# comprna/radian

Measured on AMD Instinct MI355X. Metric: signal samples/s basecalled (chunk=1024, beam=10), higher is better.
Workload: dtype f32

## Files before the change

include/radian_hip.h:

```cpp
#ifndef RADIAN_HIP_H
#define RADIAN_HIP_H

#include <stddef.h>
#include <stdint.h>

#ifdef __cplusplus
extern "C" {
#endif

#define RD_OK 0
#define RD_ERR_ARG (-1)
#define RD_ERR_HIP (-2)
#define RD_ERR_STATE (-3)
#define RD_ERR_NOMEM (-4)
#define RD_ERR_RCCL (-5)
#define RD_ERR_FORMAT (-6)
#define RD_ERR_IO (-7)
#define RD_LEN_MISSING_CONTEXT (-1)

typedef struct rd_ctx rd_ctx;

const char* rd_last_error(void);
int rd_version(void);
int rd_device_count(int* n);
int rd_decode_max_width(void);
int rd_decode_lane_width(void);

int rd_create(int device_id, rd_ctx** out);
int rd_destroy(rd_ctx* ctx);
int rd_sync(rd_ctx* ctx);
int rd_set_precision(rd_ctx* ctx, int mode);

typedef struct rd_weights_header {
    uint32_t magic;
    uint32_t version;
    uint32_t nb_filters;
    uint32_t kernel_size;
    uint32_t relu_units;
    uint32_t n_classes;
    uint32_t n_blocks;
    uint32_t dilations[16];
    uint32_t n_floats;
} rd_weights_header;
int rd_load_weights(rd_ctx* ctx, const void* blob, size_t nbytes);

int rd_load_lm(rd_ctx* ctx, const double* table, int k);
int rd_load_lm_absent(rd_ctx* ctx, int k);
int rd_load_lm_hashed(rd_ctx* ctx, const double* table, int table_order, int context_len);
int rd_set_logits(rd_ctx* ctx, int mode);
int rd_set_decode_partition(rd_ctx* ctx, int cus_per_xcd);
int rd_set_decode_math(rd_ctx* ctx, int mode);
int rd_set_head_pack(rd_ctx* ctx, int on);
int rd_head_pack_active(rd_ctx* ctx);
int64_t rd_head_pack_tiles(rd_ctx* ctx);

int rd_forward(rd_ctx* ctx, const float* windows, int n_windows, int chunk_len, float* probs);

int rd_assemble(rd_ctx* ctx, const float* probs, int n_windows, int chunk_len, int pad, int step, double* out,
                int64_t out_cap, int64_t* n_rows, int* is_f64);

int rd_decode_batch(rd_ctx* ctx, const void* probs, int prob_is_f64, const int64_t* seq_off, const int32_t* seq_len,
                    int n_seq, int beam_width, int use_lm, double s_thr, double r_thr, uint8_t* labels_out,
                    const int64_t* label_off, int32_t* label_len, double* best_score);

int rd_basecall_chunk(rd_ctx* ctx, const float* windows, int n_windows, int chunk_len, const int32_t* valid_len,
                      int beam_width, uint8_t* labels_out, int32_t* label_len);

int rd_basecall_global(rd_ctx* ctx, const float* windows, int chunk_len, int step, const int32_t* read_win_off,
                       const int32_t* pad, int n_reads, int beam_width, int use_lm, double s_thr, double r_thr,
                       uint8_t* labels_out, const int64_t* label_off, int32_t* label_len);

int rd_count_windows(int64_t n_samples, int chunk_len, int step);
int rd_basecall_reads_chunk(rd_ctx* ctx, const float* signal, const int64_t* read_off, int n_reads, int chunk_len,
                            int step, int beam_width, uint8_t* labels_out, int32_t* label_len);
int rd_basecall_reads_global(rd_ctx* ctx, const float* signal, const int64_t* read_off, int n_reads, int chunk_len,
                             int step, int beam_width, int use_lm, double s_thr, double r_thr, uint8_t* labels_out,
                             const int64_t* label_off, int32_t* label_len);

int rd_normalise_reads(rd_ctx* ctx, const int16_t* raw, const int64_t* read_off, int n_reads, int outlier_clip,
                       float* norm_out , int32_t* status);
int rd_basecall_raw_chunk(rd_ctx* ctx, const int16_t* raw, const int64_t* read_off, int n_reads, int outlier_clip,
                          int chunk_len, int step, int beam_width, uint8_t* labels_out, int32_t* label_len, int32_t* status);
int rd_basecall_raw_global(rd_ctx* ctx, const int16_t* raw, const int64_t* read_off, int n_reads, int outlier_clip,
                           int chunk_len, int step, int beam_width, int use_lm, double s_thr, double r_thr,
                           uint8_t* labels_out, const int64_t* label_off, int32_t* label_len, int32_t* status);

int rd_dev_alloc(rd_ctx* ctx, size_t bytes, void** d_ptr);
int rd_dev_free(rd_ctx* ctx, void* d_ptr);
int rd_mem_info(rd_ctx* ctx, size_t* free_bytes, size_t* total_bytes);
int rd_memcpy_h2d(rd_ctx* ctx, void* d_dst, const void* src, size_t bytes);
int rd_memcpy_d2h(rd_ctx* ctx, void* dst, const void* d_src, size_t bytes);
int rd_forward_resident(rd_ctx* ctx, const float* d_windows, int n_windows, int chunk_len, float* d_probs);
int rd_forward_reads_resident(rd_ctx* ctx, const float* d_signal, const int64_t* read_off, int n_reads, int chunk_len,
                              int step, int decode_type, int lane, int64_t* total_rows);
int rd_forward_reads(rd_ctx* ctx, const float* signal, const int64_t* read_off, int n_reads, int chunk_len, int step,
                     float* probs_out, int64_t windows_cap, int64_t* n_windows);
int rd_basecall_chunk_resident(rd_ctx* ctx, const float* d_windows, int n_windows, int chunk_len,
                               const int32_t* valid_len, int beam_width, uint8_t* labels_out, int32_t* label_len);
int rd_decode_resident(rd_ctx* ctx, const float* d_probs, int n_windows, int chunk_len, const int32_t* valid_len,
                       int beam_width, uint8_t* labels_out, int32_t* label_len);

int rd_basecall_reads_chunk_resident(rd_ctx* ctx, const float* d_signal, const int64_t* read_off, int n_reads,
                                     int chunk_len, int step, int beam_width, uint8_t* labels_out, int32_t* label_len);
int rd_basecall_reads_global_resident(rd_ctx* ctx, const float* d_signal, const int64_t* read_off, int n_reads,
                                      int chunk_len, int step, int beam_width, int use_lm, double s_thr, double r_thr,
                                      uint8_t* labels_out, const int64_t* label_off, int32_t* label_len);

int rd_pipe_config(rd_ctx* ctx, int group_batches);
int rd_pipe_set_lanes(rd_ctx* ctx, int lanes);
int rd_pipe_submit(rd_ctx* ctx, const float* d_windows, int n_windows, int chunk_len, const int32_t* valid_len,
                   int beam_width, uint8_t* labels_out, int32_t* label_len);
int rd_pipe_submit_reads(rd_ctx* ctx, const float* d_signal, const int64_t* read_off, int n_reads, int chunk_len,
                         int step, int beam_width, uint8_t* labels_out, int32_t* label_len);
int rd_pipe_submit_reads_global(rd_ctx* ctx, const float* d_signal, const int64_t* read_off, int n_reads, int chunk_len,
                                int step, int beam_width, int use_lm, double s_thr, double r_thr, uint8_t* labels_out,
                                const int64_t* label_off, int32_t* label_len);
int rd_pipe_submit_raw_global(rd_ctx* ctx, const int16_t* raw, const int64_t* read_off, int n_reads, int outlier_clip,
                              int chunk_len, int step, int beam_width, int use_lm, double s_thr, double r_thr,
                              uint8_t* labels_out, const int64_t* label_off, int32_t* label_len, int32_t* status);
int rd_pipe_submit_raw_chunk(rd_ctx* ctx, const int16_t* raw, const int64_t* read_off, int n_reads, int outlier_clip,
                             int chunk_len, int step, int beam_width, uint8_t* labels_out, int32_t* label_len, int32_t* status);
int rd_pipe_progress(rd_ctx* ctx, int64_t wait_for, int64_t* delivered);
int rd_pipe_flush(rd_ctx* ctx);
int rd_pipe_submitted(rd_ctx* ctx, int64_t* submitted);

int rd_lm_json_probe(const char* buf, size_t n, int* k_out);
int rd_lm_json_fill(const char* buf, size_t n, int k, double* table, int64_t* n_entries, int64_t* n_contexts);
int rd_lm_json_write(const char* path, const double* table, int k, int64_t* n_rows, int64_t* n_bytes);

int rd_fasta_scan(const char* buf, size_t n, int field, const char* value, uint8_t* codes, int64_t* offsets, int64_t* counts);
int rd_lm_build(rd_ctx* ctx, const uint8_t* codes, const int64_t* offsets, int64_t n_records, int k, int as_written, int unseen, double alpha,
                double r_thr, int64_t cut, double* table_out, uint32_t* counts_out, int64_t* stats);
int rd_lm_score(rd_ctx* ctx, const uint8_t* codes, const int64_t* offsets, int64_t n_records, int as_written, double r_thr, int64_t cut,
                int64_t* stats, double* nll_sum);

typedef struct rd_fast5 rd_fast5;
int rd_fast5_open(const char* path, rd_fast5** out);
int rd_fast5_open_mem(const void* buf, size_t n, rd_fast5** out);
void rd_fast5_close(rd_fast5* f);
int rd_fast5_count(const rd_fast5* f, int64_t* n_reads);
int rd_fast5_lengths(rd_fast5* f, int64_t lo, int64_t hi, int64_t* n_samples);
int rd_fast5_read_batch(rd_fast5* f, int64_t lo, int64_t hi, int16_t* samples, int64_t cap, int64_t* offsets, char* ids, int id_stride);

int rd_stitch_chunk(const uint8_t* labels, const int32_t* label_len, int chunk_len, const int32_t* read_win_off, int n_reads,
                    uint8_t* seq_out, const int64_t* seq_off, int32_t* seq_len, int n_threads);

#define RD_ALIGN_OK 0
#define RD_ALIGN_CLIP_INDEX_ERROR 1
#define RD_ALIGN_EMPTY_AFTER_CLIP 2
#define RD_ALIGN_TOO_LARGE 3
int rd_align_batch(rd_ctx* ctx, const uint8_t* refs, const int64_t* ref_off, const uint8_t* reads, const int64_t* read_off, int n_pairs,
                   int match, int mismatch, int gap_open, int gap_extend, int64_t budget_bytes, int32_t* score, int32_t* counts,
                   int32_t* status, uint8_t* ops_out, const int64_t* ops_off, int32_t* ops_len);
int64_t rd_align_workspace_bytes(int64_t n, int64_t m);
int rd_align_clip_count(const uint8_t* ops, int64_t n_ops, const uint8_t* ref, const uint8_t* read, int32_t* counts, int32_t* status);

#define RD_CTCALIGN_OK 0
#define RD_CTCALIGN_NO_PATH 1
#define RD_CTCALIGN_TOO_LARGE 2
int rd_ctc_align_batch(rd_ctx* ctx, const void* probs, int prob_is_f64, const int64_t* seq_off, const int32_t* seq_len, int n_seq,
                       const uint8_t* labels, const int64_t* label_off, const int32_t* label_len, int64_t budget_bytes,
                       int32_t* first_step, int32_t* last_step, uint8_t* qual, double* score, int32_t* status);
int64_t rd_ctc_align_workspace_bytes(int64_t n_rows, int64_t n_labels);
int rd_basecall_raw_global_q(rd_ctx* ctx, const int16_t* raw, const int64_t* read_off, int n_reads, int outlier_clip, int chunk_len,
                             int step, int beam_width, int use_lm, double s_thr, double r_thr, uint8_t* labels_out,
                             const int64_t* label_off, int32_t* label_len, int32_t* status, int64_t budget_bytes, uint8_t* qual_out,
                             int32_t* first_step_out, int32_t* last_step_out, double* score_out, int32_t* align_status);

int rd_event_stats(rd_ctx* ctx, const int16_t* raw, const int64_t* read_off, int n_reads, const int32_t* first_step,
                   const int32_t* last_step, const int64_t* label_off, const int32_t* label_len, const int32_t* align_status,
                   int32_t* ev_start, int32_t* ev_end, int64_t* ev_sum, int64_t* ev_sumsq, int16_t* ev_min, int16_t* ev_max);
int rd_event_stats_host(const int16_t* raw, const int64_t* read_off, int n_reads, const int32_t* first_step, const int32_t* last_step,
                        const int64_t* label_off, const int32_t* label_len, const int32_t* align_status, int32_t* ev_start,
                        int32_t* ev_end, int64_t* ev_sum, int64_t* ev_sumsq, int16_t* ev_min, int16_t* ev_max);
int rd_resquiggle_raw(rd_ctx* ctx, const int16_t* raw, const int64_t* read_off, int n_reads, int outlier_clip, int chunk_len, int step,
                      const uint8_t* ref_labels, const int64_t* ref_off, const int32_t* ref_len, int64_t budget_bytes,
                      int32_t* first_step, int32_t* last_step, uint8_t* qual, double* score, int32_t* align_status, int32_t* read_status,
                      int32_t* ev_start, int32_t* ev_end, int64_t* ev_sum, int64_t* ev_sumsq, int16_t* ev_min, int16_t* ev_max);

#define RD_POLYA_OK 0
#define RD_POLYA_NONE 1
#define RD_POLYA_MAD_ZERO 2
#define RD_POLYA_SHORT 3
#define RD_POLYA_EMPTY 4
#define RD_POLYA_TOO_LARGE 5
int rd_polya_segment(rd_ctx* ctx, const int16_t* raw, const int64_t* read_off, int n_reads, int win, int flat_q, int use_level, int lo_q,
                     int hi_q, int max_gap, int64_t min_samples, int64_t search_limit, int64_t budget_bytes, int32_t* status,
                     int64_t* tail_start, int64_t* tail_end, int32_t* n_flat, int64_t* sum, int64_t* sumsq, int32_t* m2, int32_t* d4,
                     int32_t* n_candidates);
int rd_polya_segment_host(const int16_t* raw, const int64_t* read_off, int n_reads, int win, int flat_q, int use_level, int lo_q, int hi_q,
                          int max_gap, int64_t min_samples, int64_t search_limit, int32_t* status, int64_t* tail_start, int64_t* tail_end,
                          int32_t* n_flat, int64_t* sum, int64_t* sumsq, int32_t* m2, int32_t* d4, int32_t* n_candidates);
int64_t rd_polya_workspace_bytes(int64_t n_samples, int win);
int rd_polya_diag_windows(rd_ctx* ctx, const int16_t* raw, const int64_t* read_off, int n_reads, int win, int flat_q, int use_level, int lo_q,
                          int hi_q, int32_t* m2, int32_t* d4, uint64_t* thr, int32_t* win_sum, int64_t* win_sumsq, uint8_t* win_flat);

#define RD_SITE_OK 0
#define RD_SITE_ONE_SIDED 1
#define RD_SITE_DEEP 2
#define RD_SITE_TOO_LARGE 3
int rd_site_compare(rd_ctx* ctx, const uint32_t* site, const uint8_t* cond, const int16_t* value, int64_t n_events, uint32_t n_sites,
                    int64_t budget_bytes, int64_t capacity, uint32_t* out_site, int32_t* status, int64_t* n, int64_t* sum, int64_t* sumsq,
                    int32_t* vmin, int32_t* vmax, int32_t* med2, int64_t* u2, int64_t* ks_num, int32_t* ks_x, int64_t* tie, int64_t* n_out);
int rd_site_compare_host(const uint32_t* site, const uint8_t* cond, const int16_t* value, int64_t n_events, uint32_t n_sites, int64_t capacity,
                         uint32_t* out_site, int32_t* status, int64_t* n, int64_t* sum, int64_t* sumsq, int32_t* vmin, int32_t* vmax,
                         int32_t* med2, int64_t* u2, int64_t* ks_num, int32_t* ks_x, int64_t* tie, int64_t* n_out);
int64_t rd_site_workspace_bytes(int64_t n_events);
// ... 172 lines not shown
```

radian_amd/_lib.py:

```python
import ctypes
import os

HERE = os.path.dirname(os.path.abspath(__file__))
LIB_PATH = os.environ.get("RADIAN_HIP_LIB") or os.path.join(HERE, "libradian_hip.so")

c_i = ctypes.c_int
c_i32p = ctypes.POINTER(ctypes.c_int32)
c_i64 = ctypes.c_int64
c_i64p = ctypes.POINTER(ctypes.c_int64)
c_d = ctypes.c_double
c_dp = ctypes.POINTER(ctypes.c_double)
c_fp = ctypes.POINTER(ctypes.c_float)
c_u8p = ctypes.POINTER(ctypes.c_uint8)
c_u32 = ctypes.c_uint32
c_u64 = ctypes.c_uint64
c_vp = ctypes.c_void_p
c_sz = ctypes.c_size_t

SIGNATURES = {
    "rd_last_error": (ctypes.c_char_p, []),
    "rd_version": (c_i, []),
    "rd_device_count": (c_i, [ctypes.POINTER(c_i)]),
    "rd_decode_max_width": (c_i, []),
    "rd_decode_lane_width": (c_i, []),
    "rd_create": (c_i, [c_i, ctypes.POINTER(c_vp)]),
    "rd_destroy": (c_i, [c_vp]),
    "rd_sync": (c_i, [c_vp]),
    "rd_set_precision": (c_i, [c_vp, c_i]),
    "rd_load_weights": (c_i, [c_vp, c_vp, c_sz]),
    "rd_load_lm": (c_i, [c_vp, c_vp, c_i]),
    "rd_load_lm_absent": (c_i, [c_vp, c_i]),
    "rd_load_lm_hashed": (c_i, [c_vp, c_vp, c_i, c_i]),
    "rd_set_logits": (c_i, [c_vp, c_i]),
    "rd_set_decode_math": (c_i, [c_vp, c_i]),
    "rd_set_head_pack": (c_i, [c_vp, c_i]),
    "rd_head_pack_active": (c_i, [c_vp]),
    "rd_head_pack_tiles": (c_i64, [c_vp]),
    "rd_set_decode_partition": (c_i, [c_vp, c_i]),
    "rd_forward": (c_i, [c_vp, c_vp, c_i, c_i, c_vp]),
    "rd_assemble": (c_i, [c_vp, c_vp, c_i, c_i, c_i, c_i, c_vp, c_i64, c_i64p, ctypes.POINTER(c_i)]),
    "rd_decode_batch": (c_i, [c_vp, c_vp, c_i, c_vp, c_vp, c_i, c_i, c_i, c_d, c_d, c_vp, c_vp, c_vp, c_vp]),
    "rd_basecall_chunk": (c_i, [c_vp, c_vp, c_i, c_i, c_vp, c_i, c_vp, c_vp]),
    "rd_basecall_global": (c_i, [c_vp, c_vp, c_i, c_i, c_vp, c_vp, c_i, c_i, c_i, c_d, c_d, c_vp, c_vp, c_vp]),
    "rd_count_windows": (c_i, [c_i64, c_i, c_i]),
    "rd_basecall_reads_chunk": (c_i, [c_vp, c_vp, c_vp, c_i, c_i, c_i, c_i, c_vp, c_vp]),
    "rd_basecall_reads_global": (c_i, [c_vp, c_vp, c_vp, c_i, c_i, c_i, c_i, c_i, c_d, c_d, c_vp, c_vp, c_vp]),
    "rd_basecall_reads_chunk_resident": (c_i, [c_vp, c_vp, c_vp, c_i, c_i, c_i, c_i, c_vp, c_vp]),
    "rd_basecall_reads_global_resident": (c_i, [c_vp, c_vp, c_vp, c_i, c_i, c_i, c_i, c_i, c_d, c_d, c_vp, c_vp, c_vp]),
    "rd_pipe_submit_reads": (c_i, [c_vp, c_vp, c_vp, c_i, c_i, c_i, c_i, c_vp, c_vp]),
    "rd_pipe_submit_reads_global": (c_i, [c_vp, c_vp, c_vp, c_i, c_i, c_i, c_i, c_i, c_d, c_d, c_vp, c_vp, c_vp]),
    "rd_pipe_submit_raw_global": (c_i, [c_vp, c_vp, c_vp, c_i, c_i, c_i, c_i, c_i, c_i, c_d, c_d, c_vp, c_vp, c_vp, c_vp]),
    "rd_pipe_submit_raw_chunk": (c_i, [c_vp, c_vp, c_vp, c_i, c_i, c_i, c_i, c_i, c_vp, c_vp, c_vp]),
    "rd_pipe_progress": (c_i, [c_vp, c_i64, c_i64p]),
    "rd_pipe_submitted": (c_i, [c_vp, c_i64p]),
    "rd_normalise_reads": (c_i, [c_vp, c_vp, c_vp, c_i, c_i, c_vp, c_vp]),
    "rd_basecall_raw_chunk": (c_i, [c_vp, c_vp, c_vp, c_i, c_i, c_i, c_i, c_i, c_vp, c_vp, c_vp]),
    "rd_basecall_raw_global": (c_i, [c_vp, c_vp, c_vp, c_i, c_i, c_i, c_i, c_i, c_i, c_d, c_d, c_vp, c_vp, c_vp, c_vp]),
    "rd_stitch_chunk": (c_i, [c_vp, c_vp, c_i, c_vp, c_i, c_vp, c_vp, c_vp, c_i]),
    "rd_fast5_open": (c_i, [ctypes.c_char_p, ctypes.POINTER(c_vp)]),
    "rd_fast5_open_mem": (c_i, [c_vp, c_sz, ctypes.POINTER(c_vp)]),
    "rd_fast5_close": (None, [c_vp]),
    "rd_fast5_count": (c_i, [c_vp, c_i64p]),
    "rd_fast5_lengths": (c_i, [c_vp, c_i64, c_i64, c_vp]),
    "rd_fast5_read_batch": (c_i, [c_vp, c_i64, c_i64, c_vp, c_i64, c_vp, c_vp, c_i]),
    "rd_lm_json_probe": (c_i, [c_vp, ctypes.c_size_t, ctypes.POINTER(c_i)]),
    "rd_lm_json_fill": (c_i, [c_vp, ctypes.c_size_t, c_i, c_vp, ctypes.POINTER(ctypes.c_int64), ctypes.POINTER(ctypes.c_int64)]),
    "rd_lm_json_write": (c_i, [ctypes.c_char_p, c_vp, c_i, c_i64p, c_i64p]),
    "rd_fasta_scan": (c_i, [c_vp, c_sz, c_i, ctypes.c_char_p, c_vp, c_vp, c_vp]),
    "rd_lm_build": (c_i, [c_vp, c_vp, c_vp, c_i64, c_i, c_i, c_i, c_d, c_d, c_i64, c_vp, c_vp, c_vp]),
    "rd_lm_score": (c_i, [c_vp, c_vp, c_vp, c_i64, c_i, c_d, c_i64, c_vp, c_dp]),
    "rd_dev_alloc": (c_i, [c_vp, c_sz, ctypes.POINTER(c_vp)]),
    "rd_mem_info": (c_i, [c_vp, ctypes.POINTER(c_sz), ctypes.POINTER(c_sz)]),
    "rd_dev_free": (c_i, [c_vp, c_vp]),
    "rd_memcpy_h2d": (c_i, [c_vp, c_vp, c_vp, c_sz]),
    "rd_memcpy_d2h": (c_i, [c_vp, c_vp, c_vp, c_sz]),
    "rd_forward_resident": (c_i, [c_vp, c_vp, c_i, c_i, c_vp]),
    "rd_forward_reads_resident": (c_i, [c_vp, c_vp, c_vp, c_i, c_i, c_i, c_i, c_i, c_vp]),
    "rd_forward_reads": (c_i, [c_vp, c_vp, c_vp, c_i, c_i, c_i, c_vp, c_i64, c_vp]),
    "rd_basecall_chunk_resident": (c_i, [c_vp, c_vp, c_i, c_i, c_vp, c_i, c_vp, c_vp]),
    "rd_decode_resident": (c_i, [c_vp, c_vp, c_i, c_i, c_vp, c_i, c_vp, c_vp]),
    "rd_pipe_config": (c_i, [c_vp, c_i]),
    "rd_pipe_set_lanes": (c_i, [c_vp, c_i]),
    "rd_pipe_submit": (c_i, [c_vp, c_vp, c_i, c_i, c_vp, c_i, c_vp, c_vp]),
    "rd_pipe_flush": (c_i, [c_vp]),
    "rd_align_batch": (c_i, [c_vp, c_vp, c_vp, c_vp, c_vp, c_i, c_i, c_i, c_i, c_i, c_i64, c_vp, c_vp, c_vp, c_vp, c_vp, c_vp]),
    "rd_align_workspace_bytes": (c_i64, [c_i64, c_i64]),
    "rd_align_clip_count": (c_i, [c_vp, c_i64, c_vp, c_vp, c_vp, c_vp]),
    "rd_ctc_align_batch": (c_i, [c_vp, c_vp, c_i, c_vp, c_vp, c_i, c_vp, c_vp, c_vp, c_i64, c_vp, c_vp, c_vp, c_vp, c_vp]),
    "rd_ctc_align_workspace_bytes": (c_i64, [c_i64, c_i64]),
    "rd_basecall_raw_global_q": (c_i, [c_vp, c_vp, c_vp, c_i, c_i, c_i, c_i, c_i, c_i, c_d, c_d, c_vp, c_vp, c_vp, c_vp, c_i64, c_vp, c_vp, c_vp, c_vp, c_vp]),
    "rd_event_stats": (c_i, [c_vp, c_vp, c_vp, c_i] + [c_vp] * 11),
    "rd_event_stats_host": (c_i, [c_vp, c_vp, c_i] + [c_vp] * 11),
    "rd_resquiggle_raw": (c_i, [c_vp, c_vp, c_vp, c_i, c_i, c_i, c_i, c_vp, c_vp, c_vp, c_i64] + [c_vp] * 12),
    "rd_polya_segment": (c_i, [c_vp, c_vp, c_vp, c_i] + [c_i] * 6 + [c_i64] * 3 + [c_vp] * 9),
    "rd_polya_segment_host": (c_i, [c_vp, c_vp, c_i] + [c_i] * 6 + [c_i64] * 2 + [c_vp] * 9),
    "rd_polya_workspace_bytes": (c_i64, [c_i64, c_i]),
    "rd_polya_diag_windows": (c_i, [c_vp, c_vp, c_vp, c_i] + [c_i] * 5 + [c_vp] * 6),
    "rd_site_compare": (c_i, [c_vp, c_vp, c_vp, c_vp, c_i64, c_u32, c_i64, c_i64] + [c_vp] * 13),
    "rd_site_compare_host": (c_i, [c_vp, c_vp, c_vp, c_i64, c_u32, c_i64] + [c_vp] * 13),
    "rd_site_workspace_bytes": (c_i64, [c_i64]),
    "rd_site_diag_segments": (c_i, [c_vp, c_vp, c_vp, c_vp, c_i64, c_u32, c_i64, c_vp, c_vp, c_vp]),
    "rd_sim_lengths": (c_i, [c_vp, c_vp, c_vp, c_i] + [c_vp] * 8 + [c_i] + [c_vp] * 4 + [c_i64, c_vp]),
    "rd_sim_lengths_host": (c_i, [c_vp, c_vp, c_i] + [c_vp] * 8 + [c_i] + [c_vp] * 4 + [c_vp]),
    "rd_sim_signal": (c_i, [c_vp, c_vp, c_vp, c_i] + [c_vp] * 8 + [c_i] + [c_vp] * 4 + [c_vp, c_i64, c_vp, c_vp, c_vp]),
    "rd_sim_signal_host": (c_i, [c_vp, c_vp, c_i] + [c_vp] * 8 + [c_i] + [c_vp] * 4 + [c_vp, c_vp, c_vp, c_vp]),
    "rd_sim_workspace_bytes": (c_i64, [c_i64, c_i64]),
    "rd_eventalign": (c_i, [c_vp, c_vp, c_vp, c_i] + [c_vp] * 7 + [c_i] + [c_vp] * 3 + [ctypes.c_int32, c_u32, ctypes.c_int32, c_i64] + [c_vp] * 13),
    "rd_eventalign_host": (c_i, [c_vp, c_vp, c_i] + [c_vp] * 7 + [c_i] + [c_vp] * 3 + [ctypes.c_int32, c_u32, ctypes.c_int32] + [c_vp] * 13),
    "rd_eventalign_workspace_bytes": (c_i64, [c_i64, c_i64]),
    "rd_sigmap": (c_i, [c_vp, c_vp, c_i64, c_i] + [c_vp] * 10 + [c_i, c_i] + [c_vp] * 3 + [c_i, c_i64] + [c_vp] * 7),
    "rd_sigmap_host": (c_i, [c_vp, c_i64, c_i] + [c_vp] * 10 + [c_i, c_i] + [c_vp] * 3 + [c_i] + [c_vp] * 7),
    "rd_sigmap_workspace_bytes": (c_i64, [c_i64, c_i64, c_i64]),
    "rd_tfrecord_open": (c_i, [ctypes.c_char_p, ctypes.POINTER(c_vp)]),
    "rd_tfrecord_open_mem": (c_i, [c_vp, c_sz, ctypes.POINTER(c_vp)]),
    "rd_tfrecord_close": (None, [c_vp]),
    "rd_tfrecord_count": (c_i, [c_vp, c_i64p, c_i64p]),
    "rd_tfrecord_read": (c_i, [c_vp, c_i64, c_i64, c_vp, c_vp, c_vp, c_vp, c_vp, c_i64]),
    "rd_crc32c": (ctypes.c_uint32, [c_vp, c_sz]),
    "rd_tfrecord_write": (c_i, [ctypes.c_char_p, c_vp, c_vp, c_vp, c_vp, c_vp, c_i64, c_i]),
    "rd_fit_batch": (c_i, [c_vp, c_vp, c_vp, c_i64, c_vp, c_vp, c_vp, c_i64, c_i, c_i, c_i, c_i, c_i64, c_vp, c_vp, c_vp, c_vp, c_vp]),
    "rd_map_minimizers": (c_i, [c_vp, c_i64, c_i, c_i, c_vp, c_vp, c_i64, c_i64p]),
    "rd_map_index": (c_i, [c_vp, c_vp, c_vp, c_i64, c_i, c_i, c_i, c_vp]),
    "rd_map_batch": (c_i, [c_vp, c_vp, c_vp, c_i64, c_i, c_i, c_i, c_i, c_i64, c_vp, c_vp, c_vp]),
    "rd_map_candidates": (c_i, [c_vp, c_vp, c_vp, c_i64, c_i, c_i, c_i, c_i, c_i64, c_i, c_i, c_i, c_vp, c_vp, c_vp, c_vp, c_vp]),
    "rd_quant_em": (c_i, [c_vp, c_vp, c_vp, c_vp, c_i64, c_i64, c_i, c_u64, c_vp, c_vp, c_vp]),
    "rd_quant_em_host": (c_i, [c_vp, c_vp, c_vp, c_i64, c_i64, c_i, c_u64, c_vp, c_vp, c_vp]),
    "rd_quant_workspace_bytes": (c_i64, [c_i64, c_i64, c_i64]),
    "rd_pileup_open": (c_i, [c_vp, c_i64]),
    "rd_pileup_close": (c_i, [c_vp]),
    "rd_pileup_add": (c_i, [c_vp, c_vp, c_vp, c_vp, c_vp, c_i, c_vp, c_i, c_i, c_i, c_i, c_i64, c_vp, c_vp, c_vp, c_vp]),
    "rd_pileup_add_ops": (c_i, [c_vp, c_vp, c_vp, c_vp, c_vp, c_vp, c_vp, c_i, c_vp, c_vp]),
    "rd_pileup_read": (c_i, [c_vp, c_u32, c_i64, c_vp, c_vp, c_vp, c_vp]),
    "rd_pileup_workspace_bytes": (c_i64, [c_i64, c_i64]),
    "rd_pileup_host": (c_i, [c_vp, c_vp, c_vp, c_vp, c_vp, c_vp, c_i, c_vp, c_i64, c_vp, c_vp, c_vp]),
    "rd_ctc_eval": (c_i, [c_vp, c_vp, c_i, c_vp, c_vp, c_vp, c_vp, c_vp, c_vp, c_vp, c_vp, c_vp]),
    "rd_ctc_probs": (c_i, [c_vp, c_vp, c_i, c_vp, c_vp, c_vp, c_vp, c_vp, c_vp, c_vp, c_vp, c_vp]),
    "rd_ctc_probs_resident": (c_i, [c_vp, c_vp, c_i, c_vp, c_vp, c_vp, c_vp, c_vp, c_vp, c_vp, c_vp, c_vp]),
    "rd_train_grad": (c_i, [c_vp, c_vp, c_i, c_vp, c_vp, c_vp, c_vp, c_vp, c_vp, c_vp]),
    "rd_train_step": (c_i, [c_vp, c_vp, c_i, c_vp, c_vp, c_vp, c_vp, c_vp, c_vp, c_vp]),
    "rd_train_step_resident": (c_i, [c_vp, c_vp, c_i, c_vp, c_vp, c_vp, c_vp, c_vp, c_vp, c_vp]),
    "rd_train_reset": (c_i, [c_vp]),
    "rd_get_weights": (c_i, [c_vp, c_vp, c_sz]),
    "rd_model_params": (c_i, [c_vp, c_i64p]),
    "rd_train_ctc_grad": (c_i, [c_vp, c_vp, c_i, c_vp, c_vp, c_vp, c_vp, c_vp, c_vp, c_vp]),
    "rd_rccl_probe": (c_i, []),
    "rd_rccl_unique_id": (c_i, [c_vp]),
    "rd_rccl_init": (c_i, [c_vp, c_i, c_i, c_vp]),
    "rd_rccl_bcast_model": (c_i, [c_vp, c_i]),
    "rd_clone_artifacts": (c_i, [c_vp, c_vp]),
    "rd_rccl_allreduce_max": (c_i, [c_vp, c_vp, c_i]),
    "rd_rccl_barrier": (c_i, [c_vp]),
    "rd_rccl_comm_count": (c_i, [c_vp, ctypes.POINTER(c_i)]),
    "rd_rccl_finalize": (c_i, [c_vp]),
}

DIAG_SIGNATURES = {
    "rd_set_conv_fuse": (c_i, [c_vp, c_i]),
    "rd_set_conv_shape": (c_i, [c_vp, c_i]),
    "rd_split3": (c_i, [c_vp, c_vp, c_sz, c_vp]),
    "rd_set_decode_form": (c_i, [c_vp, c_i]),
    "rd_pipe_policy_read": (c_i, [c_vp, c_i, c_i, c_i, c_vp, c_vp, c_vp]),
    "rd_pipe_stats": (c_i, [c_vp, c_i64p, c_i]),
    "rd_set_trie_budget": (c_i, [c_vp, c_i64]),
    "rd_map_diag_minimizers": (c_i, [c_vp, c_vp, c_vp, c_i64, c_i, c_i, c_vp, c_i64, c_i64p]),
    "rd_map_diag_chain": (c_i, [c_vp, c_vp, c_vp, c_vp, c_i64, c_i, c_i, c_i, c_i, c_vp, c_i64, c_i64p]),
    "rd_diag_score_math": (c_i, [c_vp, c_i, c_vp, c_vp, c_i64, c_vp]),
    "rd_diag_score_math_host": (c_i, [c_i, c_vp, c_vp, c_i64, c_vp]),
    "rd_timer_enable": (c_i, [c_vp, c_i, c_i]),
    "rd_timer_read": (c_i, [c_vp, c_i, c_dp, ctypes.POINTER(c_i), c_dp, c_dp]),
    "rd_timer_read_launches": (c_i, [c_vp, c_i, c_i, c_vp, c_vp, c_vp, ctypes.POINTER(c_i)]),
}

_lib = None


def load():
    global _lib
    if _lib is not None:
        return _lib
    if not os.path.exists(LIB_PATH):
        raise RuntimeError(
            f"{LIB_PATH} is missing: build it with `python -m radian_amd.build` (hipcc --offload-arch=gfx950). "
            "radian_amd has no CPU fallback.")
    lib = ctypes.CDLL(LIB_PATH)
    for name, (res, args) in {**SIGNATURES, **DIAG_SIGNATURES}.items():
        fn = getattr(lib, name)
        fn.restype = res
        fn.argtypes = args
    _lib = lib
    return lib
# ... 1 lines not shown
```

radian_amd/backend.py:

```python
import ctypes

import numpy as np

from . import _lib
from .weights import pack_blob, DEFAULT_DILATIONS

RD_TIMER_CONV, RD_TIMER_DECODE, RD_TIMER_HEAD, RD_TIMER_IN = 0, 1, 2, 3


class RadianHipError(RuntimeError):
    pass


def lib_path():
    return _lib.LIB_PATH


def _p(a):
    return None if a is None else a.ctypes.data_as(ctypes.c_void_p)


MISSING_CONTEXT = -1


# ... 692 lines not shown

    def result_raw(self):
        self.wait()
        return self.labels, self.lens, self.nw, self.status

    def result(self):
        self.wait()
        if self.decode_type == "global":
            return [_labels_of(self.labels, self.off[r], self.lens[r]) for r in range(self.n)], self.status
        return _window_labels(self.labels, self.lens, self.nw), self.status


class Backend:

    def __init__(self, device_id=0):
        self._L = _lib.load()
        h = ctypes.c_void_p()
        self._h = None
        self._check(self._L.rd_create(int(device_id), ctypes.byref(h)))
        self._h = h
        self.device_id = device_id
        self.lm_k = None
        self._tickets = {}

    def _check(self, rc):
        if rc != 0:
            raise RadianHipError(f"[rd error {rc}] " + self._L.rd_last_error().decode("utf-8", "replace"))

    def close(self):
        if self._h is not None:
            self._L.rd_destroy(self._h)
            self._h = None
        self._tickets.clear()

    def __del__(self):
        try:
            self.close()
        except Exception:
            pass

    def __enter__(self):
        return self

    def __exit__(self, *exc):
        self.close()

    def sync(self):
        self._check(self._L.rd_sync(self._h))

    def set_precision(self, mode):
        code = {"fp32": 0, "f16x3": 1, "bf16x3": 2}[mode] if isinstance(mode, str) else int(mode)
        self._check(self._L.rd_set_precision(self._h, code))

    def set_conv_shape(self, shape):
        self._check(self._L.rd_set_conv_shape(self._h, int(shape)))

    def split3(self, values):
        v = np.ascontiguousarray(values, dtype=np.float32).ravel()
        out = np.zeros((3, v.size), dtype=np.uint16)
        self._check(self._L.rd_split3(self._h, _p(v), v.size, _p(out)))
        return out

    @property
    def max_beam_width(self):
        return self._L.rd_decode_max_width()

    def load_weights(self, flat, dilations=DEFAULT_DILATIONS):
        blob = pack_blob(flat, dilations)
        self.load_weights_blob(blob)

    def load_weights_blob(self, blob):
        buf = ctypes.create_string_buffer(blob, len(blob))
        self._check(self._L.rd_load_weights(self._h, ctypes.cast(buf, ctypes.c_void_p), len(blob)))

    def load_lm(self, table, k):
        if table is None:
            self._check(self._L.rd_load_lm(self._h, None, 0))
            self.lm_k = None
            return
        table = np.ascontiguousarray(table, dtype=np.float64)
        if table.shape != (4 ** k, 4):
            raise ValueError(f"LM table must be [4^{k},4], got {table.shape}")
        self._check(self._L.rd_load_lm(self._h, _p(table), int(k)))
        self.lm_k = k

    UNSEEN = {"backoff": 0, "uniform": 1, "absent": 2}

    @staticmethod
    def _records(codes, offsets):
        codes = np.ascontiguousarray(codes, dtype=np.uint8)
        offsets = np.ascontiguousarray(offsets, dtype=np.int64)
        if offsets.ndim != 1 or len(offsets) < 1 or codes.ndim != 1 or int(offsets[-1]) != len(codes):
            raise ValueError("offsets must be [records + 1] and end at len(codes)")
        return (codes if len(codes) else np.zeros(1, dtype=np.uint8)), offsets

    def build_lm(self, codes, offsets, k, as_written=False, unseen="backoff", pseudocount=0.0, r_threshold=0.5, cut=0,
                 want_table=True, want_counts=False):
        codes, offsets = self._records(codes, offsets)
        if unseen not in self.UNSEEN:
            raise ValueError(f"unseen must be one of {sorted(self.UNSEEN)}")
        big = 1 <= k <= 13
        table = np.empty((4 ** k, 4), dtype=np.float64) if want_table and big else None
        counts = np.empty((4 ** k, 4), dtype=np.uint32) if want_counts and big else None
        st = np.zeros(32, dtype=np.int64)
        self._check(self._L.rd_lm_build(self._h, _p(codes), _p(offsets), len(offsets) - 1, int(k), 1 if as_written else 0, self.UNSEEN[unseen],
                                        float(pseudocount), float(r_threshold), int(cut), _p(table), _p(counts), _p(st)))
        self.lm_k = k
        stats = {"windows": int(st[0]), "contexts": 4 ** k, "contexts_seen": int(st[1]), "gate_contexts": int(st[2]), "gate_windows": int(st[3]),
                 "absent_rows": int(st[4]), "uniform_rows": int(st[5]), "launches": int(st[6]),
                 "stage_us": {name: int(st[24 + i]) for i, name in enumerate(("staging", "upload", "count", "table", "download"))},
                 "rows_per_order": {j: int(st[8 + j]) for j in range(k, -1, -1) if st[8 + j]}}
        if counts is not None:
            stats["counts"] = counts
        return table, stats

    def score_lm(self, codes, offsets, as_written=False, r_threshold=0.5, cut=0):
        codes, offsets = self._records(codes, offsets)
        st = np.zeros(8, dtype=np.int64)
        total = ctypes.c_double(0.0)
        self._check(self._L.rd_lm_score(self._h, _p(codes), _p(offsets), len(offsets) - 1, 1 if as_written else 0, float(r_threshold), int(cut),
                                        _p(st), ctypes.byref(total)))
        n = int(st[1])
        return {"windows": int(st[0]), "scored": n, "zero": int(st[2]), "absent": int(st[3]), "gate_windows": int(st[4]),
                "nll_sum": total.value, "mean_nll": total.value / n if n else float("nan")}

    def load_lm_absent(self, k):
        self._check(self._L.rd_load_lm_absent(self._h, int(k)))
        self.lm_k = k

    def load_lm_hashed(self, table, table_order, context_len):
        table = np.ascontiguousarray(table, dtype=np.float64)
        if table.shape != (4 ** table_order, 4):
            raise ValueError(f"LM table must be [4^{table_order},4], got {table.shape}")
        self._check(self._L.rd_load_lm_hashed(self._h, _p(table), int(table_order), int(context_len)))
        self.lm_k = context_len

    def set_logits(self, mode):
        self._check(self._L.rd_set_logits(self._h, {"f32": 0, "f16": 1}[mode] if isinstance(mode, str) else int(mode)))

    def set_trie_budget(self, nbytes):
        self._check(self._L.rd_set_trie_budget(self._h, int(nbytes)))

    def set_conv_fuse(self, on):
        self._check(self._L.rd_set_conv_fuse(self._h, 1 if on else 0))

    def set_head_pack(self, on):
        self._check(self._L.rd_set_head_pack(self._h, 1 if on else 0))

    def head_pack_active(self):
        return bool(self._L.rd_head_pack_active(self._h))

    def head_pack_tiles(self):
        return int(self._L.rd_head_pack_tiles(self._h))

    def set_decode_form(self, form):
        self._check(self._L.rd_set_decode_form(self._h, {"auto": 0, "waves": 1, "lanes": 2, "two": 3, "one": 4, "queue": 5}[form] if isinstance(form, str) else int(form)))

    def set_decode_partition(self, cus_per_xcd):
        self._check(self._L.rd_set_decode_partition(self._h, int(cus_per_xcd)))

    def set_decode_math(self, mode):
        self._check(self._L.rd_set_decode_math(self._h, {"fast": 0, "glibc": 1}[mode] if isinstance(mode, str) else int(mode)))

    def forward(self, windows):
        windows = np.ascontiguousarray(windows, dtype=np.float32)
        if windows.ndim != 2:
            raise ValueError("windows must be [n_windows, chunk_len]")
        n, T = windows.shape
        probs = np.empty((n, T, 5), dtype=np.float32)
        self._check(self._L.rd_forward(self._h, _p(windows), n, T, _p(probs)))
        return probs

    def assemble(self, probs, pad, step):
        probs = np.ascontiguousarray(probs, dtype=np.float32)
        nW, T, _ = probs.shape
        cap = (nW - 1) * step + T
        out = np.empty((max(cap, 1), 5), dtype=np.float64)
        n_rows = ctypes.c_int64(0)
        is64 = ctypes.c_int(0)
        self._check(self._L.rd_assemble(self._h, _p(probs), nW, T, int(pad), int(step), _p(out), out.shape[0],
                                        ctypes.byref(n_rows), ctypes.byref(is64)))
        out = out[: n_rows.value]
        return out if is64.value else out.astype(np.float32)

    def forward_reads(self, signals, chunk_len, step):
        flat, off = self._pack_reads(signals)
        nws = [self.count_windows(off[r + 1] - off[r], chunk_len, step) for r in range(len(signals))]
        tot = int(sum(nws))
        out = np.zeros((tot, chunk_len, 5), dtype=np.float32)
        n = ctypes.c_int64(0)
        self._check(self._L.rd_forward_reads(self._h, _p(flat), _p(off), len(signals), int(chunk_len), int(step), _p(out), tot, ctypes.byref(n)))
        assert n.value == tot
        res, w = [], 0
        for k in nws:
            res.append(out[w:w + k])
            w += k
        return res

    def decode_batch(self, mats, seq_off, seq_len, beam_width, use_lm=False, s_threshold=0.0, r_threshold=0.0,
                     with_scores=False):
        mats = np.ascontiguousarray(mats)
        if mats.dtype not in (np.float32, np.float64):
            raise TypeError("probabilities must be float32 or float64")
        seq_off = np.ascontiguousarray(seq_off, dtype=np.int64)
        seq_len = np.ascontiguousarray(seq_len, dtype=np.int32)
        n = int(seq_len.shape[0])
        label_off = np.zeros(n, dtype=np.int64)
        if n:
            label_off[1:] = np.cumsum(seq_len[:-1].astype(np.int64))
        labels = np.zeros(int(seq_len.astype(np.int64).sum()) + 1, dtype=np.uint8)
        lens = np.zeros(n, dtype=np.int32)
        scores = np.zeros(n, dtype=np.float64) if with_scores else None
        self._check(self._L.rd_decode_batch(self._h, _p(mats), 1 if mats.dtype == np.float64 else 0, _p(seq_off), _p(seq_len), n,
                                            int(beam_width), 1 if use_lm else 0, float(s_threshold), float(r_threshold),
                                            _p(labels), _p(label_off), _p(lens), _p(scores)))
        out = [_labels_of(labels, label_off[i], lens[i]) for i in range(n)]
        return (out, scores) if with_scores else out

    def decode(self, mat, beam_width, use_lm=False, s_threshold=0.0, r_threshold=0.0):
        mat = np.ascontiguousarray(mat)
        return self.decode_batch(mat.reshape(-1, 5), [0], [mat.shape[0]], beam_width, use_lm, s_threshold, r_threshold)[0]

    def basecall_chunk(self, windows, valid_len, beam_width):
        windows = np.ascontiguousarray(windows, dtype=np.float32)
        n, T = windows.shape
        valid_len = np.ascontiguousarray(valid_len, dtype=np.int32)
        labels = np.zeros((n, T), dtype=np.uint8)
        lens = np.zeros(n, dtype=np.int32)
        self._check(self._L.rd_basecall_chunk(self._h, _p(windows), n, T, _p(valid_len), int(beam_width), _p(labels), _p(lens)))
        return [labels[i, : lens[i]].copy() for i in range(n)]

    def basecall_global(self, windows, read_win_off, pads, step, beam_width, use_lm, s_threshold=0.0, r_threshold=0.0):
        windows = np.ascontiguousarray(windows, dtype=np.float32)
        nW, T = windows.shape
        read_win_off = np.ascontiguousarray(read_win_off, dtype=np.int32)
        pads = np.ascontiguousarray(pads, dtype=np.int32)
        n_reads = pads.shape[0]
        caps = np.array([(read_win_off[r + 1] - read_win_off[r] - 1) * step + T - pads[r] for r in range(n_reads)], dtype=np.int64)
        caps = np.maximum(caps, 0)
        label_off = np.zeros(n_reads, dtype=np.int64)
        label_off[1:] = np.cumsum(caps[:-1])
        labels = np.zeros(int(caps.sum()) + 1, dtype=np.uint8)
        lens = np.zeros(n_reads, dtype=np.int32)
        self._check(self._L.rd_basecall_global(self._h, _p(windows), T, int(step), _p(read_win_off), _p(pads), n_reads,
                                               int(beam_width), 1 if use_lm else 0, float(s_threshold), float(r_threshold),
                                               _p(labels), _p(label_off), _p(lens)))
        return [_labels_of(labels, label_off[r], lens[r]) for r in range(n_reads)]

    def count_windows(self, n_samples, chunk_len, step):
        n = self._L.rd_count_windows(int(n_samples), int(chunk_len), int(step))
        if n < 0:
            raise ValueError("bad window geometry")
        return n

    @staticmethod
    def _pack_reads(signals):
        return _pack(signals, np.float32)

    def basecall_reads_chunk(self, signals, chunk_len, step, beam_width):
        flat, off = self._pack_reads(signals)
        nw = [self.count_windows(off[r + 1] - off[r], chunk_len, step) for r in range(len(signals))]
        tot = int(sum(nw))
        labels = np.zeros((tot, chunk_len), dtype=np.uint8)
        lens = np.zeros(tot, dtype=np.int32)
        self._check(self._L.rd_basecall_reads_chunk(self._h, _p(flat), _p(off), len(signals), int(chunk_len), int(step),
                                                    int(beam_width), _p(labels), _p(lens)))
        return _window_labels(labels, lens, nw)

    def basecall_reads_global(self, signals, chunk_len, step, beam_width, use_lm, s_threshold=0.0, r_threshold=0.0):
        flat, off = self._pack_reads(signals)
        n = len(signals)
        labels = np.zeros(int(off[-1]) + 1, dtype=np.uint8)
        lens = np.zeros(n, dtype=np.int32)
        label_off = np.ascontiguousarray(off[:-1])
        self._check(self._L.rd_basecall_reads_global(self._h, _p(flat), _p(off), n, int(chunk_len), int(step), int(beam_width),
                                                     1 if use_lm else 0, float(s_threshold), float(r_threshold), _p(labels),
                                                     _p(label_off), _p(lens)))
        return [_labels_of(labels, off[r], lens[r]) for r in range(n)]

    STATUS_MESSAGES = {1: "MAD is zero, issue with signal.", 2: "Signal must not be empty to normalise"}

    @staticmethod
    def _pack_raw(raws):
        return _pack(raws, np.int16, pad=1)

    def normalise_reads(self, raws, outlier_clip):
        flat, off = self._pack_raw(raws)
        out = np.zeros(max(1, int(off[-1])), dtype=np.float32)
        status = np.zeros(len(raws), dtype=np.int32)
        self._check(self._L.rd_normalise_reads(self._h, _p(flat), _p(off), len(raws), int(outlier_clip), _p(out), _p(status)))
        return [out[off[r]:off[r + 1]].copy() for r in range(len(raws))], status

    def basecall_raw_chunk(self, raws, outlier_clip, chunk_len, step, beam_width):
        flat, off = self._pack_raw(raws)
        nw = [self.count_windows(off[r + 1] - off[r], chunk_len, step) for r in range(len(raws))]
        tot = int(sum(nw))
        labels = np.zeros((tot, chunk_len), dtype=np.uint8)
        lens = np.zeros(tot, dtype=np.int32)
        status = np.zeros(len(raws), dtype=np.int32)
        self._check(self._L.rd_basecall_raw_chunk(self._h, _p(flat), _p(off), len(raws), int(outlier_clip), int(chunk_len), int(step),
                                                  int(beam_width), _p(labels), _p(lens), _p(status)))
        return _window_labels(labels, lens, nw), status

    def basecall_raw_global(self, raws, outlier_clip, chunk_len, step, beam_width, use_lm, s_threshold=0.0, r_threshold=0.0):
        flat, off = self._pack_raw(raws)
        n = len(raws)
# ... 634 lines not shown
```

radian_amd/csrc/common.h:

```cpp
#pragma once
#include <hip/hip_runtime.h>
#include <stdint.h>
#include <stddef.h>
#include <string>
#include <vector>

#include "polya_rules.h"

#define RD_OK 0
#define RD_ERR_ARG (-1)
#define RD_ERR_HIP (-2)
#define RD_ERR_STATE (-3)
#define RD_ERR_NOMEM (-4)
#define RD_ERR_RCCL (-5)

void rd_set_error(const char* fmt, ...);

#define RD_HIP(expr)                                                                                   \
    do {                                                                                               \
        hipError_t _e = (expr);                                                                        \
        if (_e != hipSuccess) {                                                                        \
            rd_set_error("%s:%d: %s failed: %s", __FILE__, __LINE__, #expr, hipGetErrorString(_e));   \
            return RD_ERR_HIP;                                                                         \
        }                                                                                              \
    } while (0)

#define RD_REQUIRE(cond, ...)                                                                          \
    do {                                                                                               \
        if (!(cond)) {                                                                                 \
            rd_set_error(__VA_ARGS__);                                                                 \
            return RD_ERR_ARG;                                                                         \
        }                                                                                              \
    } while (0)

struct DevBuf {
    void* p = nullptr;
    size_t cap = 0;
    int reserve(size_t bytes);
    int reserve_exact(size_t bytes, const char* who);
    void release();
    template <typename T> T* as() const { return (T*)p; }
};

constexpr int RD_C = 256;
constexpr int RD_K = 3;
constexpr int RD_H = 128;
constexpr int RD_NCLS = 5;
constexpr int RD_MAX_BLOCKS = 16;

struct Model {
    bool loaded = false;
    int nblocks = 0;
    int dil[RD_MAX_BLOCKS] = {0};
    float* sink = nullptr;
    float* w_in = nullptr;
    float* b_in = nullptr;
    float* w_match = nullptr;
    float* b_match = nullptr;
    float* w_conv[2 * RD_MAX_BLOCKS] = {nullptr};
    float* b_conv[2 * RD_MAX_BLOCKS] = {nullptr};
    float* w_d1 = nullptr;
    float* b_d1 = nullptr;
    void* ws_conv[2 * RD_MAX_BLOCKS] = {nullptr};
    float inv_scale[2 * RD_MAX_BLOCKS] = {0};
    void* ws_d1 = nullptr;
    float inv_scale_d1 = 0.f;
    void* w3_conv[2 * RD_MAX_BLOCKS] = {nullptr};
    void* w3_d1 = nullptr;
    float* w_d2 = nullptr;
    float* b_d2 = nullptr;
    DevBuf storage;
    bool pack_ok = false;
    bool split_stale = false;
};

struct LM {
    bool loaded = false;
    int k = 0;
    int table_order = 0;
    int hashed = 0;
    double* table = nullptr;
    double* d_entropy = nullptr;
    int sparse = 0;
    uint32_t* d_missing = nullptr;
    uint32_t* gate_bits = nullptr;
    double gate_r_thr = 0.0;
    bool gate_valid = false;
    DevBuf storage, gate_storage;
};

struct TileDesc {
    int64_t seg_row;
    int64_t src_row;
    int64_t alt_row;
    int32_t t0;
    int32_t seg_len;
    int32_t in_len;
    int32_t alt_in;
    int32_t alt_res;
    int32_t pad_;
};

constexpr int RD_MAX_LAYERS = 2 * 16 + 1;

struct PackClass {
    int32_t t_lo, L, tap_lo;
    int32_t first_tile, n_tiles;
};
struct PackLayer {
    PackClass cls[3];
    int32_t n_heads;
    int32_t n_stream_tiles;
    int32_t n_tiles;
    int32_t mixed;
};
struct TileLists {
    const TileDesc* d[RD_MAX_LAYERS];
    int n[RD_MAX_LAYERS];
    int64_t rows[RD_MAX_LAYERS];
    const TileDesc* head_segs[RD_MAX_LAYERS];
    PackLayer pack[RD_MAX_LAYERS];
};

struct KernelTimer {
    bool enabled = false;
    std::vector<hipEvent_t> starts, stops;
    size_t used = 0;
    double flops = 0.0;
    double bytes = 0.0;
    std::vector<double> each_flops;
    std::vector<int> each_tag;
};

constexpr int RD_MAX_LANES = 4;
struct FwdLane {
    hipStream_t st = nullptr;
    DevBuf act[3];
    hipEvent_t done = nullptr;
};

struct rd_ctx {
    int device = 0;
    int n_cu = 256;
    int precision = 0;
    int decode_form = 0;
    int decode_math = 1;
    int conv_fuse = 1;
    int64_t packed_tiles = 0;
    int head_pack = 1;
    int conv_shape = 0;
    int logits_f16 = 0;
    hipStream_t stream = nullptr;
    hipStream_t stream_hi = nullptr;
    hipEvent_t ev_chain = nullptr;
    Model model;
    LM lm;
    DevBuf ws_tiles, ws_raw;
    int tiles_nW = -1, tiles_T = -1;
    FwdLane lanes[2 * RD_MAX_LANES];
    int part_mode = -1;
    int part_cus = 0;
    DevBuf ws_in, ws_probs, ws_mat, ws_seq, ws_nodes_child, ws_nodes_back, ws_labels, ws_misc;
    DevBuf ws_queue;
    DevBuf ws_wide, ws_wide_slot;
    DevBuf ws_align;
    DevBuf ws_ctc;
    DevBuf ws_calign;
    DevBuf ws_events, ws_events_io;
    DevBuf ws_polya, ws_polya_io;
    DevBuf ws_sim;
    DevBuf ws_eval, ws_eval_model;
    DevBuf ws_site;
    DevBuf ws_quant;
    DevBuf pileup_sites;
    DevBuf pileup_profile;
    DevBuf ws_pileup;
    int64_t pileup_n_sites = -1;
    int64_t pileup_pairs = 0;
    int64_t trie_budget = (int64_t)24 << 30;
    void* h_stage = nullptr;
    size_t h_stage_cap = 0;
    bool h_stage_busy = false;
    KernelTimer timer_conv, timer_decode, timer_head, timer_in;
    void* rccl = nullptr;
    void* rpipe = nullptr;
    int pipe_group = 4;
    int pipe_lanes = 2;
    void* plan_cache[2] = {nullptr, nullptr};
    void* train = nullptr;
    void* map = nullptr;
};

size_t rd_model_image_floats(int nblocks);
void rd_model_bind(Model& m);
int rd_model_refresh_split(rd_ctx* ctx);
int rd_model_halo(const rd_ctx* ctx);
size_t rd_lm_image_doubles(int table_order);
void rd_lm_bind(LM& lm);
int rd_lm_finish_device(rd_ctx* ctx, int table_order, int context_len, int hashed);
bool rd_pack_heads(const rd_ctx* ctx);
int rd_forward_dev(rd_ctx* ctx, const float* d_windows, int nW, int T, float* d_probs, int lane = 0);
int rd_forward_tiles_dev(rd_ctx* ctx, const float* d_signal, const TileLists& tiles, int64_t total_rows, void* d_probs, int lane = 0,
                         int probs_f16 = 0 );
int rd_lane_get(rd_ctx* ctx, int lane, FwdLane** out);
constexpr int RD_XCDS = 8;
int rd_part_set(rd_ctx* ctx, int cus_per_xcd);
int rd_masked_stream_acquire(int device, int cus_per_xcd, bool complement, hipStream_t* out);
void rd_masked_stream_release(hipStream_t st);
int rd_sync_lanes(rd_ctx* ctx);
int rd_split3_dev(rd_ctx* ctx, const float* d_in, size_t n, uint16_t* d_out);
int rd_decode_dev(rd_ctx* ctx, const void* d_probs, int ptype , const int64_t* d_seq_off, const int32_t* d_seq_len,
                  const int64_t* d_node_off, const int64_t* d_label_off, int n_seq, int64_t total_nodes, int W, int use_lm,
                  double s_thr, double r_thr, uint8_t* d_labels, int32_t* d_label_len, double* d_best_score,
                  hipStream_t stream = nullptr , const int64_t* d_seq_off2 = nullptr,
                  const int32_t* d_seq_split = nullptr, int n_cu_avail = 0 ,
                  int queue_wave_slots = 0 );
int rd_normalise_dev(rd_ctx* ctx, const int16_t* d_raw, const int64_t* d_read_off, int n_reads, int clip, float* d_out,
                     int32_t* d_status, hipStream_t stream = nullptr );
struct AsmRead {
    int64_t src_row, out_row;
    int32_t N, nW, pad, pad_;
};
int rd_assemble_batch_dev(hipStream_t st, const void* d_probs, const AsmRead* d_reads, int n_reads, int64_t max_n, int T, int step,
                          double* d_out, int streamed, int in_f16);
int rd_gather_windows_dev(hipStream_t st, const float* d_rows, const int64_t* d_off1, const int64_t* d_off2, const int32_t* d_split,
                          const int32_t* d_valid, int n_windows, int T, float* d_out);
int rd_assemble_dev(rd_ctx* ctx, const void* d_probs, int nW, int T, int pad, int step, double* d_out, int64_t N,
                    int streamed = 0 ,
                    int in_f16 = 0 );

int rd_ctc_align_dev(rd_ctx* ctx, hipStream_t st, const void* d_probs, int ptype, const int64_t* seq_off, const int32_t* seq_len, int n_seq,
                     const uint8_t* d_labels, const int64_t* dlab_off, const int32_t* label_len, int64_t budget_bytes, int32_t* first_step,
                     int32_t* last_step, uint8_t* qual, const int64_t* out_off, double* score, int32_t* status);
int rd_event_stats_dev(rd_ctx* ctx, hipStream_t st, const int16_t* d_raw, const int64_t* read_off, int n_reads, const int32_t* d_first,
                       const int32_t* d_last, const int64_t* label_off, const int32_t* label_len, const int32_t* align_status, int32_t* d_start,
                       int32_t* d_end, int64_t* d_sum, int64_t* d_sumsq, int16_t* d_min, int16_t* d_max);
int rd_event_stats_steps(rd_ctx* ctx, hipStream_t st, const int16_t* d_raw, const int64_t* read_off, int n_reads, const int32_t* first_step,
                         const int32_t* last_step, const int64_t* label_off, const int32_t* label_len, const int32_t* align_status, int64_t n_labels,
                         int32_t* ev_start, int32_t* ev_end, int64_t* ev_sum, int64_t* ev_sumsq, int16_t* ev_min, int16_t* ev_max);
int rd_polya_segment_dev(rd_ctx* ctx, hipStream_t st, const int16_t* d_raw, const int64_t* read_off, int n_reads, const PaParams& p, PaOut* d_out);
int rd_resolve_budget(int64_t* budget_bytes, size_t held);
void rd_train_invalidate(rd_ctx* ctx);
void rd_train_destroy(rd_ctx* ctx);
int rd_train_weights_host(rd_ctx* ctx, std::vector<float>& flat);
void rd_map_destroy(rd_ctx* ctx);
void rd_plan_cache_destroy_internal(rd_ctx* ctx);

bool rd_rpipe_idle(const rd_ctx* ctx);
int rd_rpipe_drain_decode(rd_ctx* ctx);
void rd_rpipe_destroy(rd_ctx* ctx);

inline bool rd_decode_len_ok(int W, int64_t rows) { return 1 + (int64_t)W * rows < ((int64_t)1 << 29); }

extern "C" int rd_decode_max_width(void);
constexpr int RD_LANE_MAX_W = 256;
constexpr int RD_HASHED_MAX_W = 64;
constexpr int RD_WIDE_MAX_W = 1024;
int rd_decode_wide_launch(rd_ctx* ctx, hipStream_t st, const void* decode_args, int ptype, int n_seq, int64_t total_nodes, bool lm);

static inline size_t align_up(size_t x, size_t a) { return (x + a - 1) / a * a; }

inline size_t rd_wide_scratch_bytes(int W)
{
    const size_t b = (size_t)2 * W * 48 + (size_t)3 * 5 * W * 8 + (size_t)2 * 5 * W * 4 + (size_t)W * 4;
    return (b + 255) & ~(size_t)255;
}

struct TrieRun {
    int k0, k1;
    int64_t nodes;
};
template <typename LenOf>
inline void rd_plan_trie_runs(const rd_ctx* ctx, int W, int k_begin, int k_end, LenOf len_of, int64_t* node_off, std::vector<TrieRun>& runs)
{
    const int64_t per_node = W > RD_LANE_MAX_W ? 24 : 20;
    const int64_t per_seq = W > RD_LANE_MAX_W ? (int64_t)rd_wide_scratch_bytes(W) : 0;
    int64_t nodes = 0, bytes = 0;
    int k0 = k_begin;
    for (int k = k_begin; k < k_end; k++) {
        const int64_t nk = 1 + (int64_t)W * len_of(k), bk = nk * per_node + per_seq;
        if (k > k0 && bytes + bk > ctx->trie_budget) {
            runs.push_back({k0, k, nodes});
            k0 = k;
            nodes = bytes = 0;
        }
        node_off[k] = nodes;
        nodes += nk;
        bytes += bk;
    }
    if (k_end > k0) runs.push_back({k0, k_end, nodes});
}

#define RD_REQUIRE_WIDTH_LM(ctx, W, use_lm)                                                                                     \
    RD_REQUIRE(!((use_lm) && (ctx)->lm.loaded && (ctx)->lm.hashed && (W) > RD_HASHED_MAX_W),                                     \
               "beam width %d with a hashed long-context RNA model (rd_load_lm_hashed): hashed contexts exist for widths up to 64", (W))
```

radian_amd/csrc/context.hip:

```cpp
#include "common.h"
#include "budget.h"
#include "../../include/radian_hip.h"
#include "../../include/radian_hip_diag.h"

#include <algorithm>
#include <stdarg.h>
#include <stdio.h>
#include <string.h>

static thread_local char g_err[1024] = "";

void rd_set_error(const char* fmt, ...)
{
    va_list ap;
    va_start(ap, fmt);
    vsnprintf(g_err, sizeof(g_err), fmt, ap);
    va_end(ap);
}

extern "C" const char* rd_last_error(void) { return g_err; }
extern "C" int rd_version(void) { return 1; }

int DevBuf::reserve(size_t bytes)
{
// ... 83 lines not shown
        return RD_ERR_HIP;
    }
    RD_REQUIRE(device_id >= 0 && device_id < n, "rd_create: device_id %d out of range [0,%d)", device_id, n);
    RD_HIP(hipSetDevice(device_id));
    hipDeviceProp_t prop;
    RD_HIP(hipGetDeviceProperties(&prop, device_id));
    if (strncmp(prop.gcnArchName, "gfx950", 6) != 0) {
        rd_set_error("rd_create: device %d is %s; libradian_hip is built for gfx950 (MI355X) only", device_id, prop.gcnArchName);
        return RD_ERR_HIP;
    }
    rd_ctx* ctx = new rd_ctx();
    ctx->device = device_id;
    ctx->n_cu = prop.multiProcessorCount > 0 ? prop.multiProcessorCount : 256;
    e = hipStreamCreateWithFlags(&ctx->stream, hipStreamNonBlocking);
    if (e == hipSuccess) {
        int lo = 0, hi = 0;
        e = hipDeviceGetStreamPriorityRange(&lo, &hi);
        if (e == hipSuccess) e = hipStreamCreateWithPriority(&ctx->stream_hi, hipStreamNonBlocking, hi);
        if (e == hipSuccess) e = hipEventCreateWithFlags(&ctx->ev_chain, hipEventDisableTiming);
    }
    if (e != hipSuccess) {
        rd_set_error("hipStreamCreate failed: %s", hipGetErrorString(e));
        if (ctx->stream) (void)hipStreamDestroy(ctx->stream);
        if (ctx->stream_hi) (void)hipStreamDestroy(ctx->stream_hi);
        delete ctx;
        return RD_ERR_HIP;
    }
    *out = ctx;
    return RD_OK;
}

static void timer_free(KernelTimer& t)
{
    for (auto ev : t.starts) (void)hipEventDestroy(ev);
    for (auto ev : t.stops) (void)hipEventDestroy(ev);
    t.starts.clear();
    t.stops.clear();
    t.each_flops.clear();
    t.each_tag.clear();
    t.used = 0;
    t.enabled = false;
}

extern "C" int rd_destroy(rd_ctx* ctx)
{
    if (!ctx) return RD_OK;
    (void)hipSetDevice(ctx->device);
    if (ctx->stream) (void)hipStreamSynchronize(ctx->stream);
    rd_rccl_finalize(ctx);
    rd_rpipe_destroy(ctx);
    rd_plan_cache_destroy_internal(ctx);
    rd_train_destroy(ctx);
    rd_map_destroy(ctx);
    timer_free(ctx->timer_conv);
    timer_free(ctx->timer_decode);
    timer_free(ctx->timer_head);
    timer_free(ctx->timer_in);
    for (int i = 0; i < 2 * RD_MAX_LANES; i++) {
        FwdLane& L = ctx->lanes[i];
        if (i > 0 && L.st) {
            (void)hipStreamSynchronize(L.st);
            if (i >= RD_MAX_LANES) rd_masked_stream_release(L.st);
            else (void)hipStreamDestroy(L.st);
        }
        if (L.done) (void)hipEventDestroy(L.done);
        for (DevBuf& b : L.act) b.release();
    }
    DevBuf* bufs[] = {&ctx->ws_tiles, &ctx->ws_raw, &ctx->ws_in, &ctx->ws_probs, &ctx->ws_mat, &ctx->ws_seq,
                      &ctx->ws_nodes_child, &ctx->ws_nodes_back, &ctx->ws_wide, &ctx->ws_wide_slot, &ctx->ws_align, &ctx->ws_ctc, &ctx->ws_calign, &ctx->ws_events, &ctx->ws_events_io, &ctx->ws_polya, &ctx->ws_polya_io, &ctx->ws_eval, &ctx->ws_eval_model, &ctx->ws_site, &ctx->ws_quant, &ctx->pileup_sites, &ctx->pileup_profile, &ctx->ws_pileup, &ctx->ws_sim, &ctx->ws_queue, &ctx->ws_labels, &ctx->ws_misc, &ctx->model.storage,
                      &ctx->lm.storage, &ctx->lm.gate_storage};
    for (DevBuf* b : bufs) b->release();
    if (ctx->h_stage) (void)hipHostFree(ctx->h_stage);
    if (ctx->stream_hi) {
        (void)hipStreamSynchronize(ctx->stream_hi);
        (void)hipStreamDestroy(ctx->stream_hi);
    }
    if (ctx->ev_chain) (void)hipEventDestroy(ctx->ev_chain);
    if (ctx->stream) (void)hipStreamDestroy(ctx->stream);
    delete ctx;
    return RD_OK;
}

extern "C" int rd_set_precision(rd_ctx* ctx, int mode)
{
    RD_REQUIRE(ctx, "rd_set_precision: null context");
    RD_REQUIRE(mode >= 0 && mode <= 2, "rd_set_precision: mode %d (0 = fp32 MFMA, 1 = split-f16 f16x3, 2 = three-term bf16x3)", mode);
    ctx->precision = mode;
    return RD_OK;
}

extern "C" int rd_sync(rd_ctx* ctx)
{
    RD_REQUIRE(ctx, "rd_sync: null context");
    return rd_sync_lanes(ctx);
}

extern "C" int rd_set_logits(rd_ctx* ctx, int mode)
{
    RD_REQUIRE(ctx, "rd_set_logits: null context");
    RD_REQUIRE(mode == 0 || mode == 1, "rd_set_logits: mode %d (0 = float32 rows, 1 = float16 rows)", mode);
    ctx->logits_f16 = mode;
    return RD_OK;
}

extern "C" int rd_set_decode_form(rd_ctx* ctx, int form)
{
    RD_REQUIRE(ctx, "rd_set_decode_form: null context");
    RD_REQUIRE(form >= 0 && form <= 5, "rd_set_decode_form: form %d (0 = per launch, 1 = waves per sequence, 2 = candidates per lane, 3 = W <= 12: two sequences per "
               "wave, 4 = one, 5 = work queue)", form);
    ctx->decode_form = form;
    return RD_OK;
}

extern "C" int rd_set_trie_budget(rd_ctx* ctx, int64_t bytes)
{
    RD_REQUIRE(ctx, "rd_set_trie_budget: null context");
    RD_REQUIRE(bytes >= 0, "rd_set_trie_budget: negative budget");
    ctx->trie_budget = bytes ? bytes : (int64_t)24 << 30;
    return RD_OK;
}

extern "C" int rd_set_conv_shape(rd_ctx* ctx, int shape)
{
    RD_REQUIRE(ctx, "rd_set_conv_shape: null context");
    RD_REQUIRE(shape == 0 || shape == 1, "rd_set_conv_shape: shape %d (0 = 128-row tiles, two workgroups per CU; 1 = 256-row tiles, one workgroup per CU)", shape);
    ctx->conv_shape = shape;
    return RD_OK;
}

extern "C" int rd_set_conv_fuse(rd_ctx* ctx, int on)
{
    RD_REQUIRE(ctx, "rd_set_conv_fuse: null context");
    RD_REQUIRE(on == 0 || on == 1, "rd_set_conv_fuse: %d (1 = block 0's first conv inside its second, 0 = its own kernel)", on);
    ctx->conv_fuse = on;
    return RD_OK;
}

extern "C" int rd_set_head_pack(rd_ctx* ctx, int on)
{
    RD_REQUIRE(ctx, "rd_set_head_pack: null context");
    RD_REQUIRE(on == 0 || on == 1, "rd_set_head_pack: %d (1 = window heads as packed classes without their zero-padding taps, 0 = as head tiles)", on);
    ctx->head_pack = on;
    return RD_OK;
}

extern "C" int rd_head_pack_active(rd_ctx* ctx)
{
    if (!ctx) return 0;
    return rd_pack_heads(ctx) ? 1 : 0;
}

extern "C" int64_t rd_head_pack_tiles(rd_ctx* ctx) { return ctx ? ctx->packed_tiles : 0; }

extern "C" int rd_set_decode_partition(rd_ctx* ctx, int cus_per_xcd)
{
    RD_REQUIRE(ctx, "rd_set_decode_partition: null context");
    RD_REQUIRE(cus_per_xcd >= -1 && cus_per_xcd <= 16, "rd_set_decode_partition: %d CUs per XCD (-1 = by beam width, 0 = off, 1..16)", cus_per_xcd);
    RD_REQUIRE(rd_rpipe_idle(ctx), "rd_set_decode_partition: pipeline not empty (call rd_pipe_flush first)");
    ctx->part_mode = cus_per_xcd;
    return RD_OK;
}

extern "C" int rd_set_decode_math(rd_ctx* ctx, int mode)
{
    RD_REQUIRE(ctx, "rd_set_decode_math: null context");
    RD_REQUIRE(mode == 0 || mode == 1, "rd_set_decode_math: mode %d (0 = library routines, 1 = glibc's operation sequence)", mode);
    ctx->decode_math = mode;
    return RD_OK;
}

extern "C" int rd_dev_alloc(rd_ctx* ctx, size_t bytes, void** d_ptr)
{
    RD_REQUIRE(ctx && d_ptr, "rd_dev_alloc: null argument");
    RD_HIP(hipSetDevice(ctx->device));
    RD_HIP(hipMalloc(d_ptr, bytes ? bytes : 1));
    return RD_OK;
}
extern "C" int rd_mem_info(rd_ctx* ctx, size_t* free_bytes, size_t* total_bytes)
{
    RD_REQUIRE(ctx && free_bytes && total_bytes, "rd_mem_info: null argument");
    RD_HIP(hipSetDevice(ctx->device));
    RD_HIP(hipMemGetInfo(free_bytes, total_bytes));
    return RD_OK;
}
extern "C" int rd_dev_free(rd_ctx* ctx, void* d_ptr)
{
    RD_REQUIRE(ctx, "rd_dev_free: null context");
    if (d_ptr) RD_HIP(hipFree(d_ptr));
    return RD_OK;
}
extern "C" int rd_memcpy_h2d(rd_ctx* ctx, void* d_dst, const void* src, size_t bytes)
{
    RD_REQUIRE(ctx && d_dst && src, "rd_memcpy_h2d: null argument");
    RD_HIP(hipMemcpyAsync(d_dst, src, bytes, hipMemcpyHostToDevice, ctx->stream));
    RD_HIP(hipStreamSynchronize(ctx->stream));
    return RD_OK;
}
extern "C" int rd_memcpy_d2h(rd_ctx* ctx, void* dst, const void* d_src, size_t bytes)
{
    RD_REQUIRE(ctx && dst && d_src, "rd_memcpy_d2h: null argument");
    RD_HIP(hipMemcpyAsync(dst, d_src, bytes, hipMemcpyDeviceToHost, ctx->stream));
    RD_HIP(hipStreamSynchronize(ctx->stream));
    return RD_OK;
}

extern "C" int rd_split3(rd_ctx* ctx, const float* values, size_t n, uint16_t* terms_out)
{
    RD_REQUIRE(ctx && values && terms_out, "rd_split3: null argument");
    RD_HIP(hipSetDevice(ctx->device));
    if (n == 0) return RD_OK;
    if (ctx->ws_in.reserve(n * 4) || ctx->ws_misc.reserve(n * 6)) return RD_ERR_NOMEM;
    RD_HIP(hipMemcpyAsync(ctx->ws_in.p, values, n * 4, hipMemcpyHostToDevice, ctx->stream));
    int rc = rd_split3_dev(ctx, ctx->ws_in.as<float>(), n, ctx->ws_misc.as<uint16_t>());
    if (rc) return rc;
    RD_HIP(hipMemcpyAsync(terms_out, ctx->ws_misc.p, n * 6, hipMemcpyDeviceToHost, ctx->stream));
    RD_HIP(hipStreamSynchronize(ctx->stream));
    return RD_OK;
}

static KernelTimer* timer_of(rd_ctx* ctx, int which)
{
    switch (which) {
        case RD_TIMER_CONV: return &ctx->timer_conv;
        case RD_TIMER_DECODE: return &ctx->timer_decode;
        case RD_TIMER_HEAD: return &ctx->timer_head;
        case RD_TIMER_IN: return &ctx->timer_in;
    }
    return nullptr;
}

extern "C" int rd_timer_enable(rd_ctx* ctx, int which, int max_launches)
{
    RD_REQUIRE(ctx, "rd_timer_enable: null context");
    KernelTimer* t = timer_of(ctx, which);
    RD_REQUIRE(t, "rd_timer_enable: unknown timer %d", which);
    RD_HIP(hipSetDevice(ctx->device));
    RD_HIP(hipStreamSynchronize(ctx->stream));
    timer_free(*t);
    t->flops = t->bytes = 0.0;
    if (max_launches <= 0) return RD_OK;
    t->starts.resize(max_launches);
    t->stops.resize(max_launches);
    for (int i = 0; i < max_launches; i++) {
        RD_HIP(hipEventCreate(&t->starts[i]));
        RD_HIP(hipEventCreate(&t->stops[i]));
    }
    t->enabled = true;
    return RD_OK;
}

extern "C" int rd_timer_read(rd_ctx* ctx, int which, double* total_ms, int* launches, double* flops, double* bytes)
{
    RD_REQUIRE(ctx, "rd_timer_read: null context");
    KernelTimer* t = timer_of(ctx, which);
    RD_REQUIRE(t, "rd_timer_read: unknown timer %d", which);
    RD_HIP(hipStreamSynchronize(ctx->stream));
    double ms = 0.0;
    for (size_t i = 0; i < t->used; i++) {
        float f = 0.f;
        RD_HIP(hipEventElapsedTime(&f, t->starts[i], t->stops[i]));
        ms += f;
    }
    if (total_ms) *total_ms = ms;
    if (launches) *launches = (int)t->used;
    if (flops) *flops = t->flops;
    if (bytes) *bytes = t->bytes;
    return RD_OK;
}

extern "C" int rd_timer_read_launches(rd_ctx* ctx, int which, int cap, float* ms_out, double* flops_out, int32_t* tag_out, int* n_out)
{
    RD_REQUIRE(ctx && n_out, "rd_timer_read_launches: null argument");
    KernelTimer* t = timer_of(ctx, which);
    RD_REQUIRE(t, "rd_timer_read_launches: unknown timer %d", which);
    RD_HIP(hipStreamSynchronize(ctx->stream));
    const size_t n = std::min(t->used, (size_t)std::max(0, cap));
    for (size_t i = 0; i < n; i++) {
        float f = 0.f;
        RD_HIP(hipEventElapsedTime(&f, t->starts[i], t->stops[i]));
        if (ms_out) ms_out[i] = f;
        if (flops_out) flops_out[i] = i < t->each_flops.size() ? t->each_flops[i] : 0.0;
        if (tag_out) tag_out[i] = i < t->each_tag.size() ? t->each_tag[i] : 0;
    }
    *n_out = (int)n;
    return RD_OK;
}
```

radian_amd/csrc/forward.hip:

```cpp
#include "common.h"

#include <algorithm>
#include <vector>
#include <mutex>

#include <stdint.h>
#include <stdlib.h>
#include <type_traits>

namespace {

typedef float f32x16 __attribute__((ext_vector_type(16)));

constexpr int BM = 128;
constexpr int BK = 16;

enum { EPI_RELU = 0, EPI_RES_IDENT = 1, EPI_RES_MATCH = 2, EPI_HEAD = 3 };

struct ZeroRows {
    uint4* row[3];
    int n16;
};
__device__ __forceinline__ void clear_zero_rows(const ZeroRows& z)
{
    if (blockIdx.x != 0) return;
    for (int r = 0; r < 3; r++)
        for (int i = threadIdx.x; i < z.n16; i += blockDim.x) z.row[r][i] = make_uint4(0u, 0u, 0u, 0u);
}

struct ConvArgs {
    const float* in;
    float* out;
    const float* wpk;
    const float* bias;
    const float* resid;
    const float* x;
    const float* wmatch;
    const float* bmatch;
    const float* w2;
    const float* b2;
    float* probs;
    int probs_f16;
    int zero_row;
    float* sink;
    const TileDesc* tiles;
    int dil;
    const float* w_in;
    const float* b_in;
    ZeroRows zr;
    const TileDesc* head_segs;
    const TileDesc* mixed;
    PackClass cls[3];
    int n_heads;
    int n_stream;
};

__device__ __forceinline__ float conv_in_value(float b, float w0, float w1, float w2, float x0, float x1, float x2)
{
    const float v = __builtin_fmaf(x2, w2, __builtin_fmaf(x1, w1, __builtin_fmaf(x0, w0, b)));
    return v > 0.f ? v : 0.f;
}

__device__ __forceinline__ void glds16_uncounted(const float* src, float* lds_dst)
{
    unsigned keep;
    const unsigned dst = (unsigned)(uintptr_t)(__attribute__((address_space(3))) void*)lds_dst;
    asm volatile("s_mov_b32 %0, m0\n\ts_mov_b32 m0, %2\n\ts_nop 0\n\tglobal_load_lds_dwordx4 %1, off\n\ts_mov_b32 m0, %0"
                 : "=&s"(keep)
                 : "v"(src), "s"(dst)
                 : "memory");
}
template <int OFFSET>
__device__ __forceinline__ void glds16_uncounted_saddr(unsigned lane_off, const void* sbase, float* lds_dst)
{
    unsigned keep;
    const unsigned dst = (unsigned)(uintptr_t)(__attribute__((address_space(3))) void*)lds_dst;
    asm volatile("s_mov_b32 %0, m0\n\ts_mov_b32 m0, %3\n\ts_nop 0\n\tglobal_load_lds_dwordx4 %1, %2 offset:%4\n\ts_mov_b32 m0, %0"
                 : "=&s"(keep)
                 : "v"(lane_off), "s"(sbase), "s"(dst), "n"(OFFSET)
                 : "memory");
}
template <int LEAVE, bool LGKM = false>
__device__ __forceinline__ void wait_dma_and_barrier()
{
    if constexpr (LGKM) asm volatile("s_waitcnt vmcnt(%0) lgkmcnt(0)\n\ts_barrier" ::"n"(LEAVE) : "memory");
    else asm volatile("s_waitcnt vmcnt(%0)\n\ts_barrier" ::"n"(LEAVE) : "memory");
}

__device__ __forceinline__ float relu_raw(float v)
{
    float r;
    asm("v_max_f32 %0, 0, %1" : "=v"(r) : "v"(v));
    return r;
}

typedef float f32x4 __attribute__((ext_vector_type(4)));
__device__ __forceinline__ __attribute__((address_space(1))) char* sgpr_base(const void* p)
{
    const uint32_t lo = __builtin_amdgcn_readfirstlane((uint32_t)(uint64_t)p), hi = __builtin_amdgcn_readfirstlane((uint32_t)((uint64_t)p >> 32));
    uint64_t u = (uint64_t)hi << 32 | lo;
    asm("" : "+s"(u));
    return (__attribute__((address_space(1))) char*)u;
}
__device__ __forceinline__ float4 gload16(const void* sbase, unsigned byte_off)
{
    asm("" : "+v"(byte_off));
    const f32x4 v = *(const __attribute__((address_space(1))) f32x4*)(sgpr_base(sbase) + byte_off);
    return make_float4(v.x, v.y, v.z, v.w);
}
__device__ __forceinline__ void gstore16(void* sbase, unsigned byte_off, float4 v)
{
    asm("" : "+v"(byte_off));
    *(__attribute__((address_space(1))) f32x4*)(sgpr_base(sbase) + byte_off) = f32x4{v.x, v.y, v.z, v.w};
}

template <int ROWS, typename Args>
__device__ __forceinline__ void head_dense5_softmax(const float* hs, const float* w2s, float* part, const TileDesc* __restrict__ tds,
                                                    const Args& a, int tid)
{
    constexpr int LDH = RD_H + 1;
    const int hrow = tid < ROWS ? tid : tid - ROWS;
    const int j0 = tid < ROWS ? 0 : RD_H / 2;
    float lg[5];
#pragma unroll
    for (int o = 0; o < 5; o++) lg[o] = tid < ROWS ? w2s[RD_H * 5 + o] : 0.f;
    for (int j = j0; j < j0 + RD_H / 2; j++) {
        const float h = hs[hrow * LDH + j];
#pragma unroll
        for (int o = 0; o < 5; o++) lg[o] += h * w2s[j * 5 + o];
    }
    if (tid >= ROWS) {
#pragma unroll
        for (int o = 0; o < 5; o++) part[hrow * 5 + o] = lg[o];
    }
    __syncthreads();
    if (tid < ROWS) {
        const TileDesc sd = tds[tid >> 5];
        const int t = sd.t0 + (tid & 31);
        const int64_t seg_row = sd.seg_row;
        if (t < sd.seg_len) {
#pragma unroll
            for (int o = 0; o < 5; o++) lg[o] += part[tid * 5 + o];
            float mx = lg[0];
#pragma unroll
            for (int o = 1; o < 5; o++) mx = lg[o] > mx ? lg[o] : mx;
            float e[5], sum = 0.f;
#pragma unroll
            for (int o = 0; o < 5; o++) {
                e[o] = expf(lg[o] - mx);
                sum += e[o];
            }
            if (a.probs_f16) {
                _Float16* pr = (_Float16*)a.probs + ((size_t)seg_row + t) * 5;
#pragma unroll
                for (int o = 0; o < 5; o++) pr[o] = (_Float16)(e[o] / sum);
            } else {
                float* pr = a.probs + ((size_t)seg_row + t) * 5;
#pragma unroll
                for (int o = 0; o < 5; o++) pr[o] = e[o] / sum;
            }
        }
    }
}

constexpr int FIN_DMAX = 2;
template <int NT, int TAPS, int EPI, int WM, bool FIN> constexpr int conv_smem_floats()
{
    constexpr int BM = 64 * WM, BN = 2 * NT * 32;
    constexpr int STAGE_FLOATS = (FIN ? 0 : BM * BK) + BN * BK;
    constexpr int HEAD_FLOATS = BM * (RD_H + 1) + RD_H * 5 + 8 + BM * 5;
    constexpr int FIN_FLOATS = FIN ? 2 * 4 * (32 + 2 * FIN_DMAX) * BK + 4 * RD_C : 0;
    return (EPI == EPI_HEAD && HEAD_FLOATS > 3 * STAGE_FLOATS) ? HEAD_FLOATS : 3 * STAGE_FLOATS + FIN_FLOATS;
}
template <int NT, int TAPS, int EPI, int WM, bool FIN, bool PACKED, int TAP_LO = 0>
__device__ __forceinline__ void tcn_gemm_tile(const ConvArgs& a, float* const smem)
{
    static_assert(!FIN || (EPI == EPI_RES_MATCH && WM == 2 && TAPS == 3 && NT == 4), "FIN: block 0's second conv, product shape");
    static_assert(!PACKED || (NT == 4 && TAPS == 3 && (EPI == EPI_RELU || EPI == EPI_RES_IDENT) && WM == 2 && !FIN), "PACKED: the product shape's conv launches behind block 0");
    constexpr int BM = 64 * WM;
    constexpr int NWAVE = 2 * WM;
    constexpr int BN = 2 * NT * 32;
    constexpr int NCHUNK = TAPS * (RD_C / BK);
    constexpr int A_FLOATS = FIN ? 0 : BM * BK;
    constexpr int STAGE_FLOATS = A_FLOATS + BN * BK;
    constexpr int HEAD_FLOATS = BM * (RD_H + 1) + RD_H * 5 + 8 + BM * 5;
    constexpr int NSTAGE = 3;
    constexpr int MIDROWS = 4 * (32 + 2 * FIN_DMAX);
    constexpr int FIN_FLOATS = FIN ? 2 * MIDROWS * BK + 4 * RD_C : 0;
    static_assert(conv_smem_floats<NT, TAPS, EPI, WM, FIN>() == ((EPI == EPI_HEAD && HEAD_FLOATS > NSTAGE * STAGE_FLOATS) ? HEAD_FLOATS : NSTAGE * STAGE_FLOATS + FIN_FLOATS),
                  "the kernel's LDS block");

    if constexpr (FIN) clear_zero_rows(a.zr);
    const int tid = threadIdx.x;
    const int lane = tid & 63;
    const int wave = __builtin_amdgcn_readfirstlane(tid >> 6);
    const int wm = wave >> 1;
    const int wn = wave & 1;
    constexpr bool PACKABLE = NT == 4 && TAPS == 3 && (EPI == EPI_RELU || EPI == EPI_RES_IDENT) && WM == 2 && !FIN;
    const TileDesc* __restrict__ tds = a.tiles + (size_t)(PACKED ? 0 : blockIdx.x) * NWAVE;
    if constexpr (PACKABLE && !PACKED) {
        if (a.mixed && (int)blockIdx.x == a.n_stream - 1) tds = a.mixed;
    }
    const TileDesc sdm[2] = {tds[wm * 2], tds[wm * 2 + 1]};
    const PackClass pkc = a.cls[TAP_LO];
    unsigned pk_p0 = 0, pk_rows = 0;
    if constexpr (PACKED) {
        pk_p0 = (unsigned)((int)blockIdx.x - pkc.first_tile) * BM;
        pk_rows = (unsigned)a.n_heads * (unsigned)pkc.L;
    }
    const bool mval[2] = {PACKED ? pk_p0 + wm * 64 < pk_rows : sdm[0].seg_len > sdm[0].t0,
                          PACKED ? pk_p0 + wm * 64 + 32 < pk_rows : sdm[1].seg_len > sdm[1].t0};

    const int dma_r = lane >> 2;
    const int dma_ps = lane & 3;
    const TileDesc sst = tds[wave];
    const int64_t d_seg = sst.seg_row, d_alt = sst.alt_row;
    const int d_t0 = sst.t0, d_ain = sst.alt_in;
    const int d_len = sst.seg_len > sst.t0 ? sst.in_len : 0;
    const int lane_slot = (dma_ps ^ ((dma_r >> 2) & 3)) * 4;
    int arow[TAPS][2];
    if constexpr (!PACKED) {
#pragma unroll
        for (int tap = 0; tap < TAPS; tap++)
#pragma unroll
            for (int pc = 0; pc < 2; pc++) {
                const int t = d_t0 + pc * 16 + dma_r - (TAPS - 1 - tap) * a.dil;
                arow[tap][pc] = (t >= 0 && t < d_len) ? (int)((t < d_ain ? d_seg : d_alt) + t) : a.zero_row;
            }
    } else {
#pragma unroll
        for (int pc = 0; pc < 2; pc++) {
            const unsigned p = pk_p0 + wave * 32 + pc * 16 + dma_r;
            const unsigned w = p / (unsigned)pkc.L;
            const int t = pkc.t_lo + (int)(p - w * (unsigned)pkc.L);
            const bool has = w < (unsigned)a.n_heads;
            const TileDesc* __restrict__ hd = a.head_segs + (has ? w : 0u);
            const int64_t h_seg = hd->seg_row, h_alt = hd->alt_row;
            const int h_len = hd->seg_len, h_in = hd->in_len, h_ain = hd->alt_in;
            const bool live = has && t < h_len;
#pragma unroll
            for (int tap = 0; tap < TAPS; tap++) {
                const int u = t - (TAPS - 1 - tap) * a.dil;
                arow[tap][pc] = (live && tap >= TAP_LO && u >= 0 && u < h_in) ? (int)((u < h_ain ? h_seg : h_alt) + u) : a.zero_row;
            }
        }
    }
    const char* lanebase = (const char*)(a.in + lane_slot);
    const unsigned lane_off = lane * 16;

    constexpr int PB = BN / (16 * NWAVE);
    constexpr int NA = FIN ? 0 : 2;
    constexpr int NPIECE = NA + PB;
    auto stage_piece_at = [&](int chunk, int cc, int ar, float* st, int pc) {
        if (pc < NA) {
            const char* src = lanebase + (size_t)cc * (BK * 4) + (uint64_t)(unsigned)ar * (RD_C * 4);
            glds16_uncounted((const float*)src, st + (wave * 2 + pc) * 256);
        } else {
            const float* wb = a.wpk + (size_t)chunk * BN * BK + wave * PB * 256;
            float* dst = st + A_FLOATS + wave * PB * 256;
            const int pb = pc - NA;
            if (pb == 0) glds16_uncounted_saddr<0>(lane_off, wb, dst);
            else if (pb == 1) glds16_uncounted_saddr<1024>(lane_off, wb, dst);
            else if (pb == 2) glds16_uncounted_saddr<2048>(lane_off, wb, dst);
            else glds16_uncounted_saddr<3072>(lane_off, wb, dst);
        }
    };
    auto stage_piece = [&](int chunk, int tap, float* st, int pc) { stage_piece_at(chunk, chunk / TAPS, arow[tap][pc & 1], st, pc); };
    auto stage = [&](int chunk, int tap, float* st) {
#pragma unroll
        for (int pc = 0; pc < NPIECE; pc++) stage_piece(chunk, tap, st, pc);
    };
    auto stage_piece_all = [&](int chunk, int cc, int tap, float* st) {
#pragma unroll
        for (int pc = 0; pc < NPIECE; pc++) stage_piece_at(chunk, cc, arow[tap][pc & 1], st, pc);
    };

    float* const midb = smem + NSTAGE * STAGE_FLOATS;
    float* const wins = midb + 2 * MIDROWS * BK;
    const int RS = 32 + 2 * a.dil;
    float xs[3][3] = {{0.f, 0.f, 0.f}, {0.f, 0.f, 0.f}, {0.f, 0.f, 0.f}};
    bool rowv[3] = {false, false, false};
    if constexpr (FIN) {
        *(float4*)(wins + tid * 4) = tid < 192 ? *(const float4*)(a.w_in + tid * 4) : *(const float4*)(a.b_in + (tid - 192) * 4);
        const float* __restrict__ xw = a.x + sst.src_row;
#pragma unroll
        for (int p = 0; p < 3; p++) {
            const int i = dma_r + 16 * p;
            const int t = d_t0 - 2 * a.dil + i;
            rowv[p] = i < RS && t >= 0 && t < d_len;
#pragma unroll
            for (int j = 0; j < 3; j++) {
                const int u = t - (2 - j) * a.dil;
                xs[p][j] = (rowv[p] && u >= 0) ? xw[u] : 0.f;
            }
        }
        __syncthreads();
    }
    auto fin_pass = [&](int cc, int p) {
        const int i = dma_r + 16 * p;
        if (i < RS) {
            const int c0 = cc * BK + dma_ps * 4;
            const float4 w0 = *(const float4*)(wins + c0), w1 = *(const float4*)(wins + RD_C + c0), w2 = *(const float4*)(wins + 2 * RD_C + c0),
                         bb = *(const float4*)(wins + 3 * RD_C + c0);
            float4 v = make_float4(0.f, 0.f, 0.f, 0.f);
            if (rowv[p]) {
                v.x = conv_in_value(bb.x, w0.x, w1.x, w2.x, xs[p][0], xs[p][1], xs[p][2]);
                v.y = conv_in_value(bb.y, w0.y, w1.y, w2.y, xs[p][0], xs[p][1], xs[p][2]);
                v.z = conv_in_value(bb.z, w0.z, w1.z, w2.z, xs[p][0], xs[p][1], xs[p][2]);
                v.w = conv_in_value(bb.w, w0.w, w1.w, w2.w, xs[p][0], xs[p][1], xs[p][2]);
            }
            const int rho = wave * RS + i;
            *(float4*)(midb + (cc & 1) * (MIDROWS * BK) + rho * BK + ((dma_ps ^ ((rho >> 2) & 3)) * 4)) = v;
        }
    };
    if constexpr (FIN) {
#pragma unroll
        for (int p = 0; p < 3; p++) fin_pass(0, p);
    }

    const int fr = lane & 31;
    const int fh = lane >> 5;
    f32x16 acc[2][NT];
#pragma unroll
    for (int n = 0; n < NT; n++) {
        const float bias = a.bias[wn * NT * 32 + n * 32 + fr];
#pragma unroll
        for (int m = 0; m < 2; m++)
#pragma unroll
            for (int e = 0; e < 16; e++) acc[m][n][e] = bias;
    }

    const int swz = (fr >> 2) & 3;
    int koff[BK / 8];
#pragma unroll
    for (int g = 0; g < BK / 8; g++) koff[g] = ((2 * g + fh) ^ swz) * 4;
    const int a_off = (wm * 64 + fr) * BK;
    const int b_off = A_FLOATS + (wn * NT * 32 + fr) * BK;

    const bool work = mval[0] || mval[1];
    int frow[3][2] = {{0, 0}, {0, 0}, {0, 0}}, fswz[3][2] = {{0, 0}, {0, 0}, {0, 0}};
    if constexpr (FIN) {
#pragma unroll
        for (int tap = 0; tap < 3; tap++)
#pragma unroll
            for (int m = 0; m < 2; m++) {
                const int rho = (wm * 2 + m) * RS + fr + tap * a.dil;
                frow[tap][m] = rho * BK;
                fswz[tap][m] = (rho >> 2) & 3;
            }
    }
    auto chunk_step = [&](const float* st, int cur, int cur_tap, const bool st_ok, int next, int next_cc, int next_ar0, int next_ar1, float* nst) {
        const float* Ab = st + a_off;
        const float* Bb = st + b_off;
        const float* Mb = midb + ((cur / TAPS) & 1) * (MIDROWS * BK);
        constexpr int NSTEP = (BK / 8) * NT;
        float4 af[2][2], bq[2];
        auto rdA = [&](int g) {
#pragma unroll
            for (int m = 0; m < 2; m++) {
                if constexpr (FIN) af[g & 1][m] = *(const float4*)(Mb + frow[cur_tap][m] + (((2 * g + fh) ^ fswz[cur_tap][m]) * 4));
                else af[g & 1][m] = *(const float4*)(Ab + m * 32 * BK + koff[g]);
            }
        };
        auto rdB = [&](int sidx) { bq[sidx & 1] = *(const float4*)(Bb + (sidx % NT) * 32 * BK + koff[sidx / NT]); };
        if (work) {
            rdA(0);
            rdB(0);
        }
#pragma unroll
        for (int sidx = 0; sidx < NSTEP; sidx++) {
            const int g = sidx / NT, n = sidx % NT;
            if (work) {
                if (sidx + 1 < NSTEP) rdB(sidx + 1);
                if (n == NT - 1 && g + 1 < BK / 8) rdA(g + 1);
#pragma unroll
                for (int kr = 0; kr < 4; kr++) {
                    const float bv = kr == 0 ? bq[sidx & 1].x : kr == 1 ? bq[sidx & 1].y : kr == 2 ? bq[sidx & 1].z : bq[sidx & 1].w;
#pragma unroll
                    for (int m = 0; m < 2; m++) {
                        const float4 aq = af[g & 1][m];
                        const float av = kr == 0 ? aq.x : kr == 1 ? aq.y : kr == 2 ? aq.z : aq.w;
                        acc[m][n] = __builtin_amdgcn_mfma_f32_32x32x2f32(av, bv, acc[m][n], 0, 0, 0);
                    }
                }
                __builtin_amdgcn_sched_group_barrier(0x100, 3, 0);
                __builtin_amdgcn_sched_group_barrier(0x008, 8, 0);
            }
            __builtin_amdgcn_sched_barrier(0);
            if (st_ok && sidx < NPIECE) stage_piece_at(next, next_cc, sidx == 0 ? next_ar0 : next_ar1, nst, sidx);
            if constexpr (FIN) {
                if (sidx == NPIECE && cur / TAPS + 1 < RD_C / BK) fin_pass(cur / TAPS + 1, cur_tap);
            }
            __builtin_amdgcn_sched_barrier(0);
        }
    };

    static_assert(NPIECE <= (BK / 8) * NT, "one DMA piece per MFMA step");
    float* st0 = smem;
    float* st1 = smem + STAGE_FLOATS;
    float* st2 = smem + 2 * STAGE_FLOATS;
    constexpr bool T3 = TAPS == 3;
    static_assert(TAPS == 3 || TAPS == 1, "tap of a chunk is a literal in the unrolled loop");
    auto step = [&](int c, int tap, const float* st, int tap2, float* nst) {
        if (c + 1 < NCHUNK) wait_dma_and_barrier<NPIECE, FIN>(); else wait_dma_and_barrier<0, FIN>();
        chunk_step(st, c, tap, c + 2 < NCHUNK, c + 2, (c + 2) / TAPS, arow[tap2][0], arow[tap2][1], nst);
    };
    auto stream_loop = [&]() {
        stage(0, 0, st0);
        stage(1, T3 ? 1 : 0, st1);
        for (int chunk = 0; chunk < NCHUNK; chunk += 3) {
            step(chunk, 0, st0, T3 ? 2 : 0, st2);
            if (chunk + 1 < NCHUNK) step(chunk + 1, T3 ? 1 : 0, st1, 0, st0);
            if (chunk + 2 < NCHUNK) step(chunk + 2, T3 ? 2 : 0, st2, T3 ? 1 : 0, st1);
        }
    };
    if constexpr (PACKED) {
        constexpr int NTP = TAPS - TAP_LO, NCH = (RD_C / BK) * NTP, PERIOD = NTP == 2 ? 6 : 3;
        stage_piece_all(TAP_LO, 0, TAP_LO, st0);
        stage_piece_all((1 / NTP) * TAPS + TAP_LO + 1 % NTP, 1 / NTP, TAP_LO + 1 % NTP, st1);
        for (int base = 0; base < NCH; base += PERIOD) {
#pragma unroll
            for (int j = 0; j < PERIOD; j++) {
                const int i = base + j;
                if (i < NCH) {
                    if (i + 1 < NCH) wait_dma_and_barrier<NPIECE>(); else wait_dma_and_barrier<0>();
                    const int tap2 = TAP_LO + (j + 2) % NTP, sl2 = base / NTP + (j + 2) / NTP;
                    chunk_step(j % 3 == 0 ? st0 : j % 3 == 1 ? st1 : st2, 0, 0, i + 2 < NCH, sl2 * TAPS + tap2, sl2, arow[tap2][0], arow[tap2][1],
                               j % 3 == 0 ? st2 : j % 3 == 1 ? st0 : st1);
                }
            }
        }
    } else {
        stream_loop();
    }
    __syncthreads();

    if constexpr (EPI != EPI_HEAD) {
        constexpr int TSTR = 64;
        float* ts = smem + wave * (32 * TSTR);
        float4* sink4 = (float4*)a.sink + (threadIdx.x & 255);
        const int rrow = lane >> 4;
        const int c4 = (lane & 15) * 4;
        auto to_patch = [&](int m, int np) {
#pragma unroll
            for (int j = 0; j < 2; j++) {
                const int n = 2 * np + j;
#pragma unroll
                for (int e = 0; e < 16; e++) {
                    const int rl = (e & 3) + 8 * (e >> 2) + 4 * fh;
                    ts[rl * TSTR + j * 32 + fr] = relu_raw(acc[m][n][e]);
                }
            }
            __builtin_amdgcn_fence(__ATOMIC_RELEASE, "wavefront");
            __builtin_amdgcn_wave_barrier();
        };
        if constexpr (PACKED) {
            {
                int2* rowinfo = (int2*)(smem + NWAVE * 32 * TSTR);
                if (tid < BM) {
                    const unsigned p = pk_p0 + tid;
                    const unsigned w = p / (unsigned)pkc.L;
                    const int t = pkc.t_lo + (int)(p - w * (unsigned)pkc.L);
                    const bool has = w < (unsigned)a.n_heads;
                    const TileDesc* __restrict__ hd = a.head_segs + (has ? w : 0u);
                    const int64_t h_seg = hd->seg_row, h_alt = hd->alt_row;
                    const bool live = has && t < hd->seg_len;
                    rowinfo[tid] = make_int2(live ? (int)(h_seg + t) : -1, live ? (int)((t < hd->alt_res ? h_seg : h_alt) + t) : a.zero_row);
                }
                __syncthreads();
#pragma unroll
                for (int m = 0; m < 2; m++) {
                    if (!mval[m]) continue;
#pragma unroll
                    for (int np = 0; np < NT / 2; np++) {
                        to_patch(m, np);
                        const int ch = wn * NT * 32 + np * 64 + c4;
#pragma unroll
                        for (int ih = 0; ih < 8; ih += 2) {
                            float4 rv[2];
                            int orow[2];
#pragma unroll
                            for (int i = 0; i < 2; i++) {
                                const int2 ri = rowinfo[wm * 64 + m * 32 + (ih + i) * 4 + rrow];
                                orow[i] = ri.x;
                                if constexpr (EPI == EPI_RES_IDENT) rv[i] = *(const float4*)(a.resid + (size_t)(unsigned)ri.y * RD_C + ch);
                            }
#pragma unroll
                            for (int i = 0; i < 2; i++) {
                                float4 v = *(const float4*)(ts + ((ih + i) * 4 + rrow) * TSTR + c4);
                                if constexpr (EPI == EPI_RES_IDENT) {
                                    v.x += rv[i].x; v.y += rv[i].y; v.z += rv[i].z; v.w += rv[i].w;
                                }
                                float4* dst = orow[i] >= 0 ? (float4*)(a.out + (size_t)(unsigned)orow[i] * RD_C + ch) : sink4;
                                *dst = v;
                            }
                        }
                        __builtin_amdgcn_fence(__ATOMIC_RELEASE, "wavefront");
                        __builtin_amdgcn_wave_barrier();
                    }
                }
                return;
            }
        }
#pragma unroll
        for (int m = 0; m < 2; m++) {
            if (!mval[m]) continue;
            const TileDesc sd = sdm[m];
            const int T = sd.seg_len;
            float* __restrict__ outw = a.out + (size_t)sd.seg_row * RD_C;
            const float* __restrict__ resw = a.resid + (size_t)sd.seg_row * RD_C;
            const float* __restrict__ resalt = a.resid + (size_t)sd.alt_row * RD_C;
            const bool interior = sd.t0 + 32 <= T;
            const bool res_one = EPI != EPI_RES_IDENT || sd.t0 + 32 <= sd.alt_res || sd.t0 >= sd.alt_res;
            if (EPI != EPI_RES_MATCH && interior && res_one) {
                const unsigned lbyte = (rrow * RD_C + c4) * 4;
                float* __restrict__ ob = outw + (size_t)sd.t0 * RD_C + wn * (NT * 32);
                const float* __restrict__ rb = (sd.t0 < sd.alt_res ? resw : resalt) + (size_t)sd.t0 * RD_C + wn * (NT * 32);
#pragma unroll
                for (int np = 0; np < NT / 2; np++) {
                    to_patch(m, np);
#pragma unroll
                    for (int ih = 0; ih < 8; ih += 4) {
                        float4 rv[4];
                        if constexpr (EPI == EPI_RES_IDENT) {
#pragma unroll
                            for (int i = 0; i < 4; i++) rv[i] = gload16(rb + np * 64 + (ih + i) * 4 * RD_C, lbyte);
                        }
#pragma unroll
                        for (int i = 0; i < 4; i++) {
                            float4 v = *(const float4*)(ts + ((ih + i) * 4 + rrow) * TSTR + c4);
                            if constexpr (EPI == EPI_RES_IDENT) {
                                v.x += rv[i].x; v.y += rv[i].y; v.z += rv[i].z; v.w += rv[i].w;
                            }
                            gstore16(ob + np * 64 + (ih + i) * 4 * RD_C, lbyte, v);
                        }
                    }
                    __builtin_amdgcn_fence(__ATOMIC_RELEASE, "wavefront");
                    __builtin_amdgcn_wave_barrier();
                }
                continue;
            }
#pragma unroll
            for (int np = 0; np < NT / 2; np++) {
                to_patch(m, np);
                const int ch = wn * NT * 32 + np * 64 + c4;
                float4 wm4 = make_float4(0.f, 0.f, 0.f, 0.f), bm4 = wm4;
                if constexpr (EPI == EPI_RES_MATCH) {
                    wm4 = *(const float4*)(a.wmatch + ch);
                    bm4 = *(const float4*)(a.bmatch + ch);
                }
                constexpr int GR = (PACKABLE && EPI == EPI_RES_IDENT) ? 2 : 4;
#pragma unroll
                for (int ih = 0; ih < 8; ih += GR) {
                    float4 rv[GR];
                    int tt[GR];
#pragma unroll
                    for (int i = 0; i < GR; i++) {
                        const int t = sd.t0 + (ih + i) * 4 + rrow;
                        tt[i] = t;
                        if constexpr (EPI == EPI_RES_IDENT) {
                            const int tc = (interior || t < T) ? t : T - 1;
                            rv[i] = *(const float4*)((tc < sd.alt_res ? resw : resalt) + (size_t)tc * RD_C + ch);
                        }
                    }
#pragma unroll
                    for (int i = 0; i < GR; i++) {
                        float4 v = *(const float4*)(ts + ((ih + i) * 4 + rrow) * TSTR + c4);
                        const int t = tt[i];
                        const bool inb = interior || t < T;
                        if constexpr (EPI == EPI_RES_IDENT) {
                            v.x += rv[i].x; v.y += rv[i].y; v.z += rv[i].z; v.w += rv[i].w;
                        } else if constexpr (EPI == EPI_RES_MATCH) {
                            const float xv = a.x[(size_t)sd.src_row + (inb ? t : T - 1)];
                            v.x = (bm4.x + xv * wm4.x) + v.x; v.y = (bm4.y + xv * wm4.y) + v.y;
                            v.z = (bm4.z + xv * wm4.z) + v.z; v.w = (bm4.w + xv * wm4.w) + v.w;
                            v.x = v.x > 0.f ? v.x : 0.f; v.y = v.y > 0.f ? v.y : 0.f;
                            v.z = v.z > 0.f ? v.z : 0.f; v.w = v.w > 0.f ? v.w : 0.f;
                        }
                        float4* dst = inb ? (float4*)(outw + (size_t)t * RD_C + ch) : sink4;
                        *dst = v;
                    }
                }
                __builtin_amdgcn_fence(__ATOMIC_RELEASE, "wavefront");
                __builtin_amdgcn_wave_barrier();
            }
        }
    } else {
        constexpr int LDH = RD_H + 1;
        float* hs = smem;
#pragma unroll
        for (int n = 0; n < NT; n++) {
            const int hcol = wn * NT * 32 + n * 32 + fr;
#pragma unroll
            for (int m = 0; m < 2; m++)
#pragma unroll
                for (int e = 0; e < 16; e++) {
                    const int row = wm * 64 + m * 32 + (e & 3) + 8 * (e >> 2) + 4 * fh;
                    const float v = acc[m][n][e];
                    hs[row * LDH + hcol] = v > 0.f ? v : 0.f;
                }
        }
        float* w2s = smem + BM * LDH;
        for (int i = tid; i < RD_H * 5; i += 64 * NWAVE) w2s[i] = a.w2[i];
        if (tid < 5) w2s[RD_H * 5 + tid] = a.b2[tid];
        __syncthreads();
        static_assert(64 * NWAVE == 2 * BM, "head epilogue: two threads per row");
        head_dense5_softmax<BM>(hs, w2s, w2s + RD_H * 5 + 8, tds, a, tid);
    }
}

template <int NT, int TAPS, int EPI, int WM, bool FIN>
__device__ __forceinline__ void tcn_gemm_workgroup(const ConvArgs& a, float* const smem)
{
    if constexpr (NT == 4 && TAPS == 3 && (EPI == EPI_RELU || EPI == EPI_RES_IDENT) && WM == 2 && !FIN) {
        const int bx = (int)blockIdx.x;
        if (bx >= a.n_stream) {
            if (bx >= a.cls[2].first_tile) tcn_gemm_tile<NT, TAPS, EPI, WM, FIN, true, 2>(a, smem);
            else if (bx >= a.cls[1].first_tile) tcn_gemm_tile<NT, TAPS, EPI, WM, FIN, true, 1>(a, smem);
            else tcn_gemm_tile<NT, TAPS, EPI, WM, FIN, true, 0>(a, smem);
            return;
        }
    }
    tcn_gemm_tile<NT, TAPS, EPI, WM, FIN, false>(a, smem);
}
template <int NT, int TAPS, int EPI, int WM = 2, bool FIN = false>
__global__ __launch_bounds__(128 * WM, WM == 2 ? 2 : 1) void tcn_gemm_kernel(ConvArgs a)
{
    __shared__ __attribute__((aligned(1024))) float smem[conv_smem_floats<NT, TAPS, EPI, WM, FIN>()];
    tcn_gemm_workgroup<NT, TAPS, EPI, WM, FIN>(a, smem);
}
template <> __global__ __launch_bounds__(256, 2) __attribute__((amdgpu_num_vgpr(92))) void tcn_gemm_kernel<4, 3, EPI_RELU, 2, false>(ConvArgs a)
{
    __shared__ __attribute__((aligned(1024))) float smem[conv_smem_floats<4, 3, EPI_RELU, 2, false>()];
    tcn_gemm_workgroup<4, 3, EPI_RELU, 2, false>(a, smem);
}
template <> __global__ __launch_bounds__(256, 2) __attribute__((amdgpu_num_vgpr(104))) void tcn_gemm_kernel<4, 3, EPI_RES_IDENT, 2, false>(ConvArgs a)
{
    __shared__ __attribute__((aligned(1024))) float smem[conv_smem_floats<4, 3, EPI_RES_IDENT, 2, false>()];
    tcn_gemm_workgroup<4, 3, EPI_RES_IDENT, 2, false>(a, smem);
}

__global__ __launch_bounds__(256) void tcn_in_kernel(const float* __restrict__ x, const float* __restrict__ w ,
                                                      const float* __restrict__ b, float* __restrict__ out,
                                                      const TileDesc* __restrict__ tiles, int dil, ZeroRows zr)
{
    clear_zero_rows(zr);
    const TileDesc td = tiles[(size_t)blockIdx.x * 4 + (threadIdx.x >> 6)];
    const int c4 = (threadIdx.x & 63) * 4;
    const float4 w0 = *(const float4*)(w + c4), w1 = *(const float4*)(w + 256 + c4), w2 = *(const float4*)(w + 512 + c4);
    const float4 bb = *(const float4*)(b + c4);
    const float* xw = x + td.src_row;
    float* ow = out + (size_t)td.seg_row * RD_C;
    const int tend = td.t0 + 32 < td.seg_len ? td.t0 + 32 : td.seg_len;
    for (int t = td.t0; t < tend; t++) {
        const float x2 = xw[t];
        const float x1 = t - dil >= 0 ? xw[t - dil] : 0.f;
        const float x0 = t - 2 * dil >= 0 ? xw[t - 2 * dil] : 0.f;
        float4 v;
        v.x = conv_in_value(bb.x, w0.x, w1.x, w2.x, x0, x1, x2);
        v.y = conv_in_value(bb.y, w0.y, w1.y, w2.y, x0, x1, x2);
        v.z = conv_in_value(bb.z, w0.z, w1.z, w2.z, x0, x1, x2);
        v.w = conv_in_value(bb.w, w0.w, w1.w, w2.w, x0, x1, x2);
        *(float4*)(ow + (size_t)t * RD_C + c4) = v;
    }
}

typedef _Float16 f16x8 __attribute__((ext_vector_type(8)));
typedef _Float16 f16x4 __attribute__((ext_vector_type(4)));
constexpr int ROWH = 2 * RD_C;

struct SplitArgs {
    const _Float16* in;
    _Float16* out;
    const _Float16* wpk;
    const float* bias;
    float inv_scale;
    const _Float16* resid;
    const float* x;
    const float* wmatch;
    const float* bmatch;
    const float* w2;
    const float* b2;
    float* probs;
    int probs_f16;
    int zero_row;
    float* sink;
    const TileDesc* tiles;
    int dil;
};

template <int NT, int TAPS, int EPI>
__global__ __launch_bounds__(256, 2) void tcn_gemm_split_kernel(SplitArgs a)
{
    constexpr int BN = 2 * NT * 32;
    constexpr int BKC = 16;
    constexpr int NCHUNK = TAPS * (RD_C / BKC);
    constexpr int STAGE_FLOATS = (BM + BN) * 16;
    constexpr int NSTAGE = 3;
    constexpr int HEAD_FLOATS = BM * (RD_H + 1) + RD_H * 5 + 8 + BM * 5;
    constexpr int SMEM_FLOATS = (EPI == EPI_HEAD && HEAD_FLOATS > NSTAGE * STAGE_FLOATS) ? HEAD_FLOATS : NSTAGE * STAGE_FLOATS;

    __shared__ __attribute__((aligned(1024))) float smem[SMEM_FLOATS];

    const int tid = threadIdx.x;
    const int lane = tid & 63;
    const int wave = __builtin_amdgcn_readfirstlane(tid >> 6);
    const int wm = wave >> 1;
    const int wn = wave & 1;
    const TileDesc* __restrict__ tds = a.tiles + (size_t)blockIdx.x * 4;
    const TileDesc sdm[2] = {tds[wm * 2], tds[wm * 2 + 1]};
    const bool mval[2] = {sdm[0].seg_len > sdm[0].t0, sdm[1].seg_len > sdm[1].t0};

    const int dma_r = lane >> 2;
    const int dma_ps = lane & 3;
    const TileDesc sst = tds[wave];
    const int64_t d_seg = sst.seg_row, d_alt = sst.alt_row;
    const int d_t0 = sst.t0, d_ain = sst.alt_in;
    const int d_len = sst.seg_len > sst.t0 ? sst.in_len : 0;
    const int lslot = dma_ps ^ ((dma_r >> 2) & 3);
    const int lane_half = (lslot & 1) * 8 + (lslot >> 1) * 32;
    int arow[TAPS][2];
#pragma unroll
    for (int tap = 0; tap < TAPS; tap++)
#pragma unroll
        for (int pc = 0; pc < 2; pc++) {
            const int t = d_t0 + pc * 16 + dma_r - (TAPS - 1 - tap) * a.dil;
            arow[tap][pc] = (t >= 0 && t < d_len) ? (int)((t < d_ain ? d_seg : d_alt) + t) : a.zero_row;
        }
    const char* lanebase = (const char*)(a.in + lane_half);
    const unsigned lane_off = lane * 16;

    constexpr int PB = BN / 64;
    constexpr int NPIECE = 2 + PB;
    auto stage_piece = [&](int chunk, int tap, float* st, int pc) {
        if (pc < 2) {
            const int cc = chunk / TAPS;
            const char* src = lanebase + (size_t)((cc >> 1) * 128 + (cc & 1) * 32) + (uint64_t)(unsigned)arow[tap][pc] * (ROWH * 2);
            glds16_uncounted((const float*)src, st + (wave * 2 + pc) * 256);
        } else {
            const float* wb = (const float*)(a.wpk + (size_t)chunk * BN * 32) + wave * PB * 256;
            float* dst = st + BM * 16 + wave * PB * 256;
            if (pc == 2) glds16_uncounted_saddr<0>(lane_off, wb, dst);
            else if (pc == 3) glds16_uncounted_saddr<1024>(lane_off, wb, dst);
            else if (pc == 4) glds16_uncounted_saddr<2048>(lane_off, wb, dst);
            else glds16_uncounted_saddr<3072>(lane_off, wb, dst);
        }
    };
    auto stage = [&](int chunk, int tap, float* st) {
#pragma unroll
        for (int pc = 0; pc < NPIECE; pc++) stage_piece(chunk, tap, st, pc);
    };

    const int fr = lane & 31;
    const int fh = lane >> 5;
    f32x16 acc[2][NT];
#pragma unroll
    for (int n = 0; n < NT; n++) {
        const float bias = a.bias[wn * NT * 32 + n * 32 + fr] / a.inv_scale;
#pragma unroll
        for (int m = 0; m < 2; m++)
#pragma unroll
            for (int e = 0; e < 16; e++) acc[m][n][e] = bias;
    }

    const int swz = (fr >> 2) & 3;
    const int oh = (fh ^ swz) * 8;
    const int ol = ((2 + fh) ^ swz) * 8;
    const int a_off = (wm * 64 + fr) * 32;
    const int b_off = BM * 32 + (wn * NT * 32 + fr) * 32;

    const bool work = mval[0] || mval[1];
    auto chunk_step = [&](const float* stf, int next, int next_tap, float* nst) {
        const _Float16* st = (const _Float16*)stf;
// ... 431 lines not shown
                int tt[8];
#pragma unroll
                for (int i = 0; i < 8; i++) {
                    const int t = sd.t0 + i * 4 + rrow;
                    tt[i] = t;
                    if constexpr (EPI == EPI_RES_IDENT) {
                        const int tc = (interior || t < T) ? t : T - 1;
                        const __bf16* rb = (tc < sd.alt_res ? resw : resalt) + (size_t)tc * ROW3 + hoff;
#pragma unroll
                        for (int q = 0; q < 3; q++) r3[i][q] = *(const bf16x4*)(rb + 16 * q);
                    }
                }
#pragma unroll
                for (int i = 0; i < 8; i++) {
                    const float4 p = *(const float4*)(ts + (i * 4 + rrow) * TSTR + c4);
                    float v[4] = {p.x, p.y, p.z, p.w};
                    const int t = tt[i];
                    const bool inb = interior || t < T;
                    if constexpr (EPI == EPI_RES_IDENT) {
#pragma unroll
                        for (int q = 0; q < 4; q++) {
                            v[q] += (float)r3[i][0][q] + ((float)r3[i][1][q] + (float)r3[i][2][q]);
                            v[q] = v[q] > 0.f ? v[q] : 0.f;
                        }
                    } else if constexpr (EPI == EPI_RES_MATCH) {
                        const float xv = a.x[(size_t)sd.src_row + (inb ? t : T - 1)];
                        const float wq[4] = {wm4.x, wm4.y, wm4.z, wm4.w}, bq[4] = {bm4.x, bm4.y, bm4.z, bm4.w};
#pragma unroll
                        for (int q = 0; q < 4; q++) {
                            v[q] = (bq[q] + xv * wq[q]) + v[q];
                            v[q] = v[q] > 0.f ? v[q] : 0.f;
                        }
                    }
                    bf16x4 o3[3];
#pragma unroll
                    for (int q = 0; q < 4; q++) {
                        __bf16 h, md, l;
                        split3(v[q], h, md, l);
                        o3[0][q] = h;
                        o3[1][q] = md;
                        o3[2][q] = l;
                    }
                    __bf16* ob = outw + (size_t)t * ROW3 + hoff;
#pragma unroll
                    for (int q = 0; q < 3; q++) {
                        bf16x4* d = inb ? (bf16x4*)(ob + 16 * q) : sinkh;
                        *d = o3[q];
                    }
                }
                __builtin_amdgcn_fence(__ATOMIC_RELEASE, "wavefront");
                __builtin_amdgcn_wave_barrier();
            }
        }
    } else {
        constexpr int LDH = RD_H + 1;
        float* hs = smem;
#pragma unroll
        for (int n = 0; n < NT; n++) {
            const int hcol = wn * NT * 32 + n * 32 + fr;
#pragma unroll
            for (int m = 0; m < 2; m++)
#pragma unroll
                for (int e = 0; e < 16; e++) {
                    const int row = wm * 64 + m * 32 + (e & 3) + 8 * (e >> 2) + 4 * fh;
                    const float v = acc[m][n][e];
                    hs[row * LDH + hcol] = v > 0.f ? v : 0.f;
                }
        }
        float* w2s = smem + BM3 * LDH;
        for (int i = tid; i < RD_H * 5; i += 512) w2s[i] = a.w2[i];
        if (tid < 5) w2s[RD_H * 5 + tid] = a.b2[tid];
        __syncthreads();
        head_dense5_softmax<BM3>(hs, w2s, w2s + RD_H * 5 + 8, tds, a, tid);
    }
}

__global__ __launch_bounds__(256) void tcn_in_bf3_kernel(const float* __restrict__ x, const float* __restrict__ w, const float* __restrict__ b,
                                                          __bf16* __restrict__ out, const TileDesc* __restrict__ tiles, int dil, ZeroRows zr)
{
    clear_zero_rows(zr);
    const TileDesc td = tiles[(size_t)blockIdx.x * 4 + (threadIdx.x >> 6)];
    const int c4 = (threadIdx.x & 63) * 4;
    const float4 w0 = *(const float4*)(w + c4), w1 = *(const float4*)(w + 256 + c4), w2 = *(const float4*)(w + 512 + c4);
    const float4 bb = *(const float4*)(b + c4);
    const float* xw = x + td.src_row;
    __bf16* ow = out + (size_t)td.seg_row * ROW3;
    const int hoff = (c4 >> 4) * 48 + (c4 & 15);
    const int tend = td.t0 + 32 < td.seg_len ? td.t0 + 32 : td.seg_len;
    for (int t = td.t0; t < tend; t++) {
        const float x2 = xw[t];
        const float x1 = t - dil >= 0 ? xw[t - dil] : 0.f;
        const float x0 = t - 2 * dil >= 0 ? xw[t - 2 * dil] : 0.f;
        float v[4];
        v[0] = bb.x + x0 * w0.x + x1 * w1.x + x2 * w2.x;
        v[1] = bb.y + x0 * w0.y + x1 * w1.y + x2 * w2.y;
        v[2] = bb.z + x0 * w0.z + x1 * w1.z + x2 * w2.z;
        v[3] = bb.w + x0 * w0.w + x1 * w1.w + x2 * w2.w;
        bf16x4 o3[3];
#pragma unroll
        for (int q = 0; q < 4; q++) {
            const float r = v[q] > 0.f ? v[q] : 0.f;
            __bf16 h, md, l;
            split3(r, h, md, l);
            o3[0][q] = h;
            o3[1][q] = md;
            o3[2][q] = l;
        }
#pragma unroll
        for (int q = 0; q < 3; q++) *(bf16x4*)(ow + (size_t)t * ROW3 + hoff + 16 * q) = o3[q];
    }
}

__global__ void split3_kernel(const float* __restrict__ v, uint16_t* __restrict__ out, size_t n)
{
    const size_t i = (size_t)blockIdx.x * blockDim.x + threadIdx.x;
    if (i >= n) return;
    __bf16 h, m, l;
    split3(v[i], h, m, l);
    out[i] = *(const uint16_t*)&h;
    out[n + i] = *(const uint16_t*)&m;
    out[2 * n + i] = *(const uint16_t*)&l;
}

int timer_begin(hipStream_t st, KernelTimer& tm)
{
    if (tm.enabled && tm.used < tm.starts.size()) RD_HIP(hipEventRecord(tm.starts[tm.used], st));
    return RD_OK;
}
int timer_end(hipStream_t st, KernelTimer& tm, double flops, double bytes, int tag = 0)
{
    if (tm.enabled && tm.used < tm.starts.size()) {
        RD_HIP(hipEventRecord(tm.stops[tm.used], st));
        tm.used++;
        tm.flops += flops;
        tm.bytes += bytes;
        tm.each_flops.push_back(flops);
        tm.each_tag.push_back(tag);
    }
    return RD_OK;
}

}

namespace {

bool fuse_first_conv(const rd_ctx* ctx)
{
    return ctx->conv_fuse && ctx->precision == 0 && ctx->conv_shape == 0 && ctx->model.nblocks >= 1 && ctx->model.dil[0] >= 1 &&
           ctx->model.dil[0] <= FIN_DMAX;
}

int launch_layer(rd_ctx* ctx, hipStream_t st, int b, int kind , const TileDesc* tiles, int n,
                double rows, int zero_row, const float* d_signal, float* Xin, float* Xout, float* MID, float* d_probs, int probs_f16,
                const PackLayer* pk, const TileDesc* head_segs)
{
    if (n <= 0) return RD_OK;
    Model& m = ctx->model;
    const bool split = ctx->precision == 1;
    const bool bf3 = ctx->precision == 2;
    if (kind != 0 && (bf3 || (!split && ctx->conv_shape == 1)))
        RD_REQUIRE(n % 2 == 0, "internal: %d tiles in a layer of 256-row workgroups (lists are padded to pairs)", n);
    int rc;
    ZeroRows zr = {};
    const bool fin = kind == 2 && b == 0 && fuse_first_conv(ctx);
    if (kind == 0 || fin) {
        const size_t row_bytes = (size_t)RD_C * (bf3 ? 6 : 4);
        zr.n16 = (int)(row_bytes / 16);
        zr.row[0] = (uint4*)((char*)Xin + (size_t)zero_row * row_bytes);
        zr.row[1] = (uint4*)((char*)Xout + (size_t)zero_row * row_bytes);
        zr.row[2] = (uint4*)((char*)MID + (size_t)zero_row * row_bytes);
    }
    if (kind == 0 && fuse_first_conv(ctx)) return RD_OK;
    if (bf3) {
        Bf3Args h = {};
        h.zero_row = zero_row;
        h.sink = m.sink;
        h.tiles = tiles;
        if (kind == 0) {
            if ((rc = timer_begin(st, ctx->timer_in))) return rc;
            hipLaunchKernelGGL(tcn_in_bf3_kernel, dim3(n), dim3(256), 0, st, d_signal, m.w_in, m.b_in, (__bf16*)MID, tiles, m.dil[0], zr);
            RD_HIP(hipGetLastError());
            return timer_end(st, ctx->timer_in, 2.0 * rows * RD_C * RD_K, rows * (RD_C * 6.0 + 4.0));
        }
        if (kind == 3) {
            if ((rc = timer_begin(st, ctx->timer_head))) return rc;
            h.in = (const __bf16*)Xin;
            h.wpk = (const __bf16*)m.w3_d1;
            h.bias = m.b_d1;
            h.w2 = m.w_d2;
            h.b2 = m.b_d2;
            h.probs = d_probs;
            h.probs_f16 = probs_f16;
            hipLaunchKernelGGL((tcn_gemm_bf3_kernel<2, 1, EPI_HEAD>), dim3(n / 2), dim3(512), 0, st, h);
            RD_HIP(hipGetLastError());
            return timer_end(st, ctx->timer_head, 2.0 * rows * (RD_C * RD_H + RD_H * 5), rows * (RD_C * 6.0 + 20.0));
        }
        const int wi = 2 * b + (kind == 2 ? 1 : 0);
        h.dil = m.dil[b];
        h.wpk = (const __bf16*)m.w3_conv[wi];
        h.bias = m.b_conv[wi];
        if (kind == 1) {
            h.in = (const __bf16*)Xin;
            h.out = (__bf16*)MID;
        } else {
            h.in = (const __bf16*)MID;
            h.out = (__bf16*)Xout;
            h.resid = (const __bf16*)Xin;
            h.x = d_signal;
            h.wmatch = m.w_match;
            h.bmatch = m.b_match;
        }
        if ((rc = timer_begin(st, ctx->timer_conv))) return rc;
        if (kind == 1) hipLaunchKernelGGL((tcn_gemm_bf3_kernel<4, 3, EPI_RELU>), dim3(n / 2), dim3(512), 0, st, h);
        else if (b == 0) hipLaunchKernelGGL((tcn_gemm_bf3_kernel<4, 3, EPI_RES_MATCH>), dim3(n / 2), dim3(512), 0, st, h);
        else hipLaunchKernelGGL((tcn_gemm_bf3_kernel<4, 3, EPI_RES_IDENT>), dim3(n / 2), dim3(512), 0, st, h);
        RD_HIP(hipGetLastError());
        return timer_end(st, ctx->timer_conv, 2.0 * rows * RD_C * RD_C * RD_K, (kind == 2 && b > 0 ? 3.0 : 2.0) * rows * RD_C * 6.0, kind == 1 ? 0 : b == 0 ? 2 : 1);
    }
    if (kind == 0) {
        if ((rc = timer_begin(st, ctx->timer_in))) return rc;
        if (split)
            hipLaunchKernelGGL(tcn_in_split_kernel, dim3(n), dim3(256), 0, st, d_signal, m.w_in, m.b_in, (_Float16*)MID, tiles, m.dil[0], zr);
        else
            hipLaunchKernelGGL(tcn_in_kernel, dim3(n), dim3(256), 0, st, d_signal, m.w_in, m.b_in, MID, tiles, m.dil[0], zr);
        RD_HIP(hipGetLastError());
        return timer_end(st, ctx->timer_in, 2.0 * rows * RD_C * RD_K, rows * (RD_C * 4.0 + 4.0));
    }
    if (kind == 3) {
        if ((rc = timer_begin(st, ctx->timer_head))) return rc;
        if (split) {
            SplitArgs h = {};
            h.zero_row = zero_row;
            h.sink = m.sink;
            h.tiles = tiles;
            h.in = (const _Float16*)Xin;
            h.wpk = (const _Float16*)m.ws_d1;
            h.inv_scale = m.inv_scale_d1;
            h.bias = m.b_d1;
            h.w2 = m.w_d2;
            h.b2 = m.b_d2;
            h.probs = d_probs;
            h.probs_f16 = probs_f16;
            hipLaunchKernelGGL((tcn_gemm_split_kernel<2, 1, EPI_HEAD>), dim3(n), dim3(256), 0, st, h);
        } else {
            ConvArgs h = {};
            h.zero_row = zero_row;
            h.sink = m.sink;
            h.tiles = tiles;
            h.in = Xin;
            h.wpk = m.w_d1;
            h.bias = m.b_d1;
            h.w2 = m.w_d2;
            h.b2 = m.b_d2;
            h.probs = d_probs;
            h.probs_f16 = probs_f16;
            if (ctx->conv_shape == 1) hipLaunchKernelGGL((tcn_gemm_kernel<2, 1, EPI_HEAD, 4>), dim3(n / 2), dim3(512), 0, st, h);
            else hipLaunchKernelGGL((tcn_gemm_kernel<2, 1, EPI_HEAD>), dim3(n), dim3(256), 0, st, h);
        }
        RD_HIP(hipGetLastError());
        return timer_end(st, ctx->timer_head, 2.0 * rows * (RD_C * RD_H + RD_H * 5), rows * (RD_C * 4.0 + 20.0));
    }
    const int wi = 2 * b + (kind == 2 ? 1 : 0);
    ConvArgs a = {};
    a.zero_row = zero_row;
    a.sink = m.sink;
    a.dil = m.dil[b];
    a.tiles = tiles;
    a.wpk = m.w_conv[wi];
    a.bias = m.b_conv[wi];
    a.n_stream = INT32_MAX;
    if (b > 0 && pk && head_segs && pk->n_tiles > 0 && rd_pack_heads(ctx)) {
        a.head_segs = head_segs;
        a.mixed = pk->mixed ? head_segs + pk->n_heads : nullptr;
        for (int c = 0; c < 3; c++) a.cls[c] = pk->cls[c];
        a.n_heads = pk->n_heads;
        a.n_stream = pk->n_stream_tiles;
        n = pk->n_tiles;
        ctx->packed_tiles += pk->n_tiles - pk->n_stream_tiles;
    }
    SplitArgs sa = {};
    sa.zero_row = zero_row;
    sa.sink = m.sink;
    sa.dil = m.dil[b];
    sa.tiles = tiles;
    sa.wpk = (const _Float16*)m.ws_conv[wi];
    sa.inv_scale = m.inv_scale[wi];
    sa.bias = m.b_conv[wi];
    if (kind == 1) {
        a.in = Xin;
        a.out = MID;
        sa.in = (const _Float16*)Xin;
        sa.out = (_Float16*)MID;
    } else {
        a.in = MID;
        a.out = Xout;
        a.resid = Xin;
        a.x = d_signal;
        a.wmatch = m.w_match;
        a.bmatch = m.b_match;
        sa.in = (const _Float16*)MID;
        sa.out = (_Float16*)Xout;
        sa.resid = (const _Float16*)Xin;
        sa.x = d_signal;
        sa.wmatch = m.w_match;
        sa.bmatch = m.b_match;
    }
    if ((rc = timer_begin(st, ctx->timer_conv))) return rc;
    if (kind == 1) {
        if (split) hipLaunchKernelGGL((tcn_gemm_split_kernel<4, 3, EPI_RELU>), dim3(n), dim3(256), 0, st, sa);
        else if (ctx->conv_shape == 1) hipLaunchKernelGGL((tcn_gemm_kernel<4, 3, EPI_RELU, 4>), dim3(n / 2), dim3(512), 0, st, a);
        else hipLaunchKernelGGL((tcn_gemm_kernel<4, 3, EPI_RELU>), dim3(n), dim3(256), 0, st, a);
    } else if (b == 0) {
        if (fin) {
            a.w_in = m.w_in;
            a.b_in = m.b_in;
            a.zr = zr;
            a.in = nullptr;
        }
        if (split) hipLaunchKernelGGL((tcn_gemm_split_kernel<4, 3, EPI_RES_MATCH>), dim3(n), dim3(256), 0, st, sa);
        else if (ctx->conv_shape == 1) hipLaunchKernelGGL((tcn_gemm_kernel<4, 3, EPI_RES_MATCH, 4>), dim3(n / 2), dim3(512), 0, st, a);
        else if (fin) hipLaunchKernelGGL((tcn_gemm_kernel<4, 3, EPI_RES_MATCH, 2, true>), dim3(n), dim3(256), 0, st, a);
        else hipLaunchKernelGGL((tcn_gemm_kernel<4, 3, EPI_RES_MATCH>), dim3(n), dim3(256), 0, st, a);
    } else {
        if (split) hipLaunchKernelGGL((tcn_gemm_split_kernel<4, 3, EPI_RES_IDENT>), dim3(n), dim3(256), 0, st, sa);
        else if (ctx->conv_shape == 1) hipLaunchKernelGGL((tcn_gemm_kernel<4, 3, EPI_RES_IDENT, 4>), dim3(n / 2), dim3(512), 0, st, a);
        else hipLaunchKernelGGL((tcn_gemm_kernel<4, 3, EPI_RES_IDENT>), dim3(n), dim3(256), 0, st, a);
    }
    RD_HIP(hipGetLastError());
    return timer_end(st, ctx->timer_conv, 2.0 * rows * RD_C * RD_C * RD_K, (kind == 2 && b > 0 ? 3.0 : 2.0) * rows * RD_C * 4.0, kind == 1 ? 0 : b == 0 ? 2 : 1);
}

}

bool rd_pack_heads(const rd_ctx* ctx)
{
    return ctx->head_pack && ctx->precision == 0 && ctx->conv_shape == 0 && ctx->model.loaded && ctx->model.pack_ok;
}

int rd_split3_dev(rd_ctx* ctx, const float* d_in, size_t n, uint16_t* d_out)
{
    if (n == 0) return RD_OK;
    hipLaunchKernelGGL(split3_kernel, dim3((unsigned)((n + 255) / 256)), dim3(256), 0, ctx->stream, d_in, d_out, n);
    RD_HIP(hipGetLastError());
    return RD_OK;
}

namespace {
struct MaskedStream {
    int device, cus;
    bool complement, in_use;
    hipStream_t st;
};
std::vector<MaskedStream> g_masked;
std::mutex g_masked_mu;
}

int rd_masked_stream_acquire(int device, int cus_per_xcd, bool complement, hipStream_t* out)
{
    std::lock_guard<std::mutex> lk(g_masked_mu);
    for (MaskedStream& m : g_masked)
        if (!m.in_use && m.device == device && m.cus == cus_per_xcd && m.complement == complement) {
            m.in_use = true;
            *out = m.st;
            return RD_OK;
        }
    uint32_t mask[RD_XCDS] = {0};
    const int nbits = RD_XCDS * 32, k = RD_XCDS * cus_per_xcd;
    for (int i = 0; i < nbits; i++)
        if ((i < k) != complement) mask[i / 32] |= 1u << (i % 32);
    hipStream_t st = nullptr;
    RD_HIP(hipExtStreamCreateWithCUMask(&st, RD_XCDS, mask));
    g_masked.push_back({device, cus_per_xcd, complement, true, st});
    *out = st;
    return RD_OK;
}

void rd_masked_stream_release(hipStream_t st)
{
    if (!st) return;
    (void)hipStreamSynchronize(st);
    std::lock_guard<std::mutex> lk(g_masked_mu);
    for (MaskedStream& m : g_masked)
        if (m.st == st) m.in_use = false;
}

int rd_lane_get(rd_ctx* ctx, int lane, FwdLane** out)
{
    if (lane < 0 || lane >= 2 * RD_MAX_LANES) {
        rd_set_error("forward lane %d out of range", lane);
        return RD_ERR_ARG;
    }
    FwdLane& L = ctx->lanes[lane];
    if (!L.st) {
        if (lane == 0) L.st = ctx->stream;
        else if (lane < RD_MAX_LANES) {
            RD_HIP(hipStreamCreateWithFlags(&L.st, hipStreamNonBlocking));
        }
        else {
            if (ctx->part_cus < 1 || ctx->part_cus > 31) {
                rd_set_error("internal: partitioned lane %d without a decode partition", lane);
                return RD_ERR_STATE;
            }
            int rc = rd_masked_stream_acquire(ctx->device, ctx->part_cus, true, &L.st);
            if (rc) return rc;
        }
    }
    if (!L.done) RD_HIP(hipEventCreateWithFlags(&L.done, hipEventDisableTiming));
    *out = &L;
    return RD_OK;
}

int rd_part_set(rd_ctx* ctx, int cus_per_xcd)
{
    if (ctx->part_cus == cus_per_xcd) return RD_OK;
    for (int i = RD_MAX_LANES; i < 2 * RD_MAX_LANES; i++) {
        FwdLane& L = ctx->lanes[i];
        if (L.st) {
            rd_masked_stream_release(L.st);
            L.st = nullptr;
        }
    }
    ctx->part_cus = cus_per_xcd;
    return RD_OK;
}

int rd_sync_lanes(rd_ctx* ctx)
{
    RD_HIP(hipStreamSynchronize(ctx->stream));
    for (int i = 1; i < 2 * RD_MAX_LANES; i++)
        if (ctx->lanes[i].st) RD_HIP(hipStreamSynchronize(ctx->lanes[i].st));
    return RD_OK;
}

int rd_forward_tiles_dev(rd_ctx* ctx, const float* d_signal, const TileLists& tl, int64_t total_rows, void* d_probs, int lane, int probs_f16)
{
    Model& m = ctx->model;
    if (!m.loaded) {
        rd_set_error("rd_forward: no weights loaded (rd_load_weights)");
        return RD_ERR_STATE;
    }
    if (total_rows == 0) return RD_OK;
    int rc = RD_OK;
    if (m.split_stale && ctx->precision != 0 && (rc = rd_model_refresh_split(ctx))) return rc;
    FwdLane* L = nullptr;
    if ((rc = rd_lane_get(ctx, lane, &L))) return rc;
    if (total_rows >= INT32_MAX) {
        rd_set_error("rd_forward: %lld rows in one batch (the kernels index rows with 32 bits)", (long long)total_rows);
        return RD_ERR_ARG;
    }
    const size_t row_bytes = (size_t)RD_C * (ctx->precision == 2 ? 6 : 4);
    const size_t act_bytes = (size_t)(total_rows + 1) * row_bytes;
    if (L->act[0].reserve(act_bytes) || L->act[1].reserve(act_bytes) || L->act[2].reserve(act_bytes)) return RD_ERR_NOMEM;
    float* Xin = L->act[0].as<float>();
    float* Xout = L->act[1].as<float>();
    float* MID = L->act[2].as<float>();
    const int zero_row = (int)total_rows;
    const int nl = 2 * m.nblocks + 1;
    ctx->packed_tiles = 0;
    for (int li = 0; li < nl; li++) {
        const int b = li == nl - 1 ? m.nblocks : li / 2;
        const int kind = li == nl - 1 ? 3 : (li == 0 ? 0 : (li & 1 ? 2 : 1));
        if ((rc = launch_layer(ctx, L->st, b, kind, tl.d[li], tl.n[li], (double)tl.rows[li], zero_row, d_signal, Xin, Xout, MID, (float*)d_probs, probs_f16,
                               &tl.pack[li], tl.head_segs[li])))
            return rc;
        if (kind == 2) {
            float* t = Xin;
            Xin = Xout;
            Xout = t;
        }
    }
    RD_HIP(hipEventRecord(L->done, L->st));
    return RD_OK;
}

int rd_uniform_tiles(rd_ctx* ctx, int nW, int T, TileLists* out)
{
    const int subs = (T + 31) / 32;
    const size_t nsub = (size_t)nW * subs;
    const size_t n = (nsub + 7) / 8 * 2;
    if (ctx->tiles_nW != nW || ctx->tiles_T != T) {
        std::vector<TileDesc> h(n * 4);
        for (size_t i = 0; i < n * 4; i++) {
            TileDesc& td = h[i];
            const size_t w = i / subs;
            const int k = (int)(i % subs);
            const bool real = i < nsub;
            td.seg_row = real ? (int64_t)w * T : 0;
            td.src_row = td.seg_row;
            td.alt_row = td.seg_row;
            td.t0 = real ? k * 32 : 0;
            td.seg_len = real ? T : 0;
            td.in_len = td.seg_len;
            td.alt_in = INT32_MAX;
            td.alt_res = INT32_MAX;
            td.pad_ = 0;
        }
        if (ctx->ws_tiles.reserve(h.size() * sizeof(TileDesc))) return RD_ERR_NOMEM;
        if (int rcs = rd_sync_lanes(ctx)) return rcs;
        RD_HIP(hipMemcpy(ctx->ws_tiles.p, h.data(), h.size() * sizeof(TileDesc), hipMemcpyHostToDevice));
        ctx->tiles_nW = nW;
        ctx->tiles_T = T;
    }
    const int nl = 2 * ctx->model.nblocks + 1;
    for (int li = 0; li < RD_MAX_LAYERS; li++) {
        out->d[li] = li < nl ? ctx->ws_tiles.as<TileDesc>() : nullptr;
        out->n[li] = li < nl ? (int)n : 0;
        out->rows[li] = li < nl ? (int64_t)nW * T : 0;
        out->head_segs[li] = nullptr;
        out->pack[li] = PackLayer();
    }
    return RD_OK;
}

int rd_forward_dev(rd_ctx* ctx, const float* d_windows, int nW, int T, float* d_probs, int lane)
{
    RD_REQUIRE(nW >= 0 && T >= 1, "rd_forward: bad shape nW=%d T=%d", nW, T);
    if (nW == 0) return RD_OK;
    if (!ctx->model.loaded) {
        rd_set_error("rd_forward: no weights loaded (rd_load_weights)");
        return RD_ERR_STATE;
    }
    TileLists tl;
    int rc = rd_uniform_tiles(ctx, nW, T, &tl);
    if (rc) return rc;
    return rd_forward_tiles_dev(ctx, d_windows, tl, (int64_t)nW * T, d_probs, lane);
}
```

radian_amd/csrc/plan.hip:

```cpp
#include "plan.h"

#include <string.h>

namespace rdi {

int64_t assembled_rows(int nW, int T, int pad, int step)
{
    int64_t N = 0;
    for (int i = 0; i < nW; i++) {
        int rows = (i == nW - 1) ? T - pad : T;
        int64_t end = (int64_t)i * step + rows;
        if (rows > 0 && end > N) N = end;
    }
    return N;
}

int assembled_is_f64(int nW, int T, int pad, int step)
{
    if (step >= T) return 0;
    if (nW >= 3) return 1;
    if (nW == 2 && T - pad > 0) return 1;
    return 0;
}

// ... 66 lines not shown
            segs.push_back(j < nS ? list[j] : e);
        }
    }
    const int t1 = d < h ? d : h, t2 = 2 * d < h ? 2 * d : h;
    const int lo[3] = {t2, t1, 0}, hi[3] = {h, t2, t1};
    int32_t tile = pk.n_stream_tiles;
    for (int c = 0; c < 3; c++) {
        PackClass& pc = pk.cls[c];
        pc.t_lo = lo[c];
        pc.L = hi[c] - lo[c];
        pc.tap_lo = c;
        pc.first_tile = tile;
        pc.n_tiles = (int32_t)((nH * pc.L + 127) / 128);
        tile += pc.n_tiles;
    }
    pk.n_tiles = tile;
}

int plan_reads_chunk(const Model& m, const int64_t* read_off, int n_reads, int chunk, int step, int halo, ReadsPlan& P)
{
    LayerHalo lh[RD_MAX_LAYERS];
    layer_halos(m, lh);
    P.n_layers = 2 * m.nblocks + 1;
    P.per_layer = true;
    int64_t row = 0;
    P.read_win_off.assign(1, 0);
    std::vector<TileDesc> heads[RD_MAX_LAYERS];
    for (int r = 0; r < n_reads; r++) {
        const int64_t N = read_off[r + 1] - read_off[r];
        RD_REQUIRE(N >= 1, "read %d is empty", r);
        RD_REQUIRE(N < INT32_MAX, "read %d too long", r);
        const WindowGeom g = window_geom(N, chunk, step);
        const int64_t stream_row = row;
        P.read_row.push_back(stream_row);
        for (int li = 0; li < P.n_layers; li++) add_segment(P.tiles[li], P.rows[li], stream_row, read_off[r], (int)N, (int)N);
        row += N;
        for (int i = 0; i < g.nW; i++) {
            const int valid = (i < g.nW - 1) ? chunk : chunk - g.pad;
            const int h = (i == 0) ? 0 : (halo < valid ? halo : valid);
            int64_t o1 = stream_row + (int64_t)i * step;
            if (h > 0) {
                o1 = row;
                const int64_t alt = stream_row + (int64_t)i * step;
                for (int li = 0; li < P.n_layers; li++) {
                    const int len = lh[li].h_out < valid ? lh[li].h_out : valid;
                    if (len > 0)
                        add_segment(heads[li], P.rows[li], row, read_off[r] + (int64_t)i * step, len, valid, alt, lh[li].h_in, lh[li].h_res);
                }
                row += h;
            }
            P.off1.push_back(o1);
            P.off2.push_back(stream_row + (int64_t)i * step);
            P.split.push_back(h);
            P.valid.push_back(valid);
        }
        P.n_windows += g.nW;
        P.read_win_off.push_back(P.n_windows);
    }
    for (int li = 2; li < P.n_layers - 1; li++)
        pack_layer_heads(P.tiles[li], heads[li], m.dil[li / 2], lh[li].h_out < chunk ? lh[li].h_out : chunk, P.head_segs[li], P.pack[li]);
    for (int li = 0; li < P.n_layers; li++) P.tiles[li].insert(P.tiles[li].end(), heads[li].begin(), heads[li].end());
    P.total_rows = row;
    return RD_OK;
}

int plan_reads_global(const Model& m, const int64_t* read_off, int n_reads, int chunk, int step, int halo, ReadsPlan& P, bool* streamed)
{
    const bool st = step <= chunk - halo;
    *streamed = st;
    P.n_layers = 2 * m.nblocks + 1;
    P.per_layer = false;
    int64_t row = 0;
    P.read_win_off.assign(1, 0);
    for (int r = 0; r < n_reads; r++) {
        const int64_t N = read_off[r + 1] - read_off[r];
        RD_REQUIRE(N >= 1, "read %d is empty", r);
        RD_REQUIRE(N < INT32_MAX, "read %d too long", r);
        const WindowGeom g = window_geom(N, chunk, step);
        P.read_row.push_back(row);
        if (st) {
            add_segment(P.tiles[0], P.rows[0], row, read_off[r], (int)N, (int)N);
            row += N;
        } else {
            for (int i = 0; i < g.nW; i++) {
                const int valid = (i < g.nW - 1) ? chunk : chunk - g.pad;
                if (valid > 0) add_segment(P.tiles[0], P.rows[0], row + (int64_t)i * chunk, read_off[r] + (int64_t)i * step, valid, valid);
            }
            row += (int64_t)g.nW * chunk;
        }
        P.valid.push_back(g.pad);
        P.n_windows += g.nW;
        P.read_win_off.push_back(P.n_windows);
    }
    P.total_rows = row;
    return RD_OK;
}

size_t plan_pad_tiles(ReadsPlan& P)
{
    size_t total = 0;
    for (int li = 0; li < P.n_layers; li++)
        if (P.per_layer || li == 0) {
            std::vector<TileDesc>& v = P.tiles[li];
            while (v.size() % 8) {
                TileDesc e = {};
                e.alt_in = e.alt_res = INT32_MAX;
                v.push_back(e);
            }
            total += v.size();
        }
    return total;
}

bool PlanKey::matches(const Model& m, const int64_t* read_off, int n_reads, int chunk_, int step_, int mode_, int halo_) const
{
    if (!valid || chunk != chunk_ || step != step_ || mode != mode_ || halo != halo_ || nblocks != m.nblocks || read_off[0] != 0 ||
        lens.size() != (size_t)n_reads)
        return false;
    for (int b = 0; b < m.nblocks; b++)
        if (dil[b] != m.dil[b]) return false;
    for (int r = 0; r < n_reads; r++)
        if (lens[r] != read_off[r + 1] - read_off[r]) return false;
    return true;
}

int PlanKey::rebuild(const Model& m, const int64_t* read_off, int n_reads, int chunk_, int step_, int mode_, int halo_, ReadsPlan& P, bool* streamed,
                     size_t* n_desc)
{
    invalidate();
    P = ReadsPlan();
    int rc = mode_ == 0 ? plan_reads_chunk(m, read_off, n_reads, chunk_, step_, halo_, P) : plan_reads_global(m, read_off, n_reads, chunk_, step_, halo_, P, streamed);
    if (rc) return rc;
    *n_desc = plan_pad_tiles(P);
    chunk = chunk_;
    step = step_;
    mode = mode_;
    halo = halo_;
    nblocks = m.nblocks;
    for (int b = 0; b < RD_MAX_BLOCKS; b++) dil[b] = b < m.nblocks ? m.dil[b] : 0;
    lens.resize(n_reads);
    for (int r = 0; r < n_reads; r++) lens[r] = read_off[r + 1] - read_off[r];
    return RD_OK;
}

size_t plan_fill_lists(const ReadsPlan& P, const TileDesc* d_base, TileDesc* h_dst, TileLists& lists)
{
    size_t off = 0;
    for (int li = 0; li < RD_MAX_LAYERS; li++) {
        lists.d[li] = nullptr;
        lists.n[li] = 0;
        lists.rows[li] = 0;
        lists.head_segs[li] = nullptr;
        lists.pack[li] = PackLayer();
    }
    for (int li = 0; li < P.n_layers; li++) {
        if (P.per_layer || li == 0) {
            const std::vector<TileDesc>& v = P.tiles[li];
            if (!v.empty()) memcpy(h_dst + off, v.data(), v.size() * sizeof(TileDesc));
            lists.d[li] = d_base + off;
            lists.n[li] = (int)(v.size() / 4);
            lists.rows[li] = P.rows[li];
            off += v.size();
        } else {
            lists.d[li] = lists.d[0];
            lists.n[li] = lists.n[0];
            lists.rows[li] = lists.rows[0];
        }
    }
    return off;
}

size_t plan_packed_descs(const ReadsPlan& P)
{
    size_t n = 0;
    for (int li = 0; li < RD_MAX_LAYERS; li++) n += P.head_segs[li].size();
    return n;
}

size_t plan_fill_packed(const ReadsPlan& P, const TileDesc* d_base, TileDesc* h_dst, TileLists& lists)
{
    size_t off = 0;
    for (int li = 0; li < RD_MAX_LAYERS; li++) {
        const std::vector<TileDesc>& v = P.head_segs[li];
        lists.head_segs[li] = nullptr;
        lists.pack[li] = PackLayer();
        if (v.empty() || P.pack[li].n_tiles == 0) continue;
        memcpy(h_dst + off, v.data(), v.size() * sizeof(TileDesc));
        lists.head_segs[li] = d_base + off;
        lists.pack[li] = P.pack[li];
        off += v.size();
    }
    return off;
}

int pinned_reserve(void** p, size_t* cap, size_t bytes)
{
    if (bytes <= *cap) return RD_OK;
    if (*p) (void)hipHostFree(*p);
    *p = nullptr;
    *cap = 0;
    size_t want = align_up(bytes + bytes / 8, 1 << 16);
    RD_HIP(hipHostMalloc(p, want, hipHostMallocDefault));
    *cap = want;
    return RD_OK;
}

}
```

Before: 27.66 million.

## Stage conv input rows once per channel slice as shared slab across taps

Adds a SLAB variant of the TCN conv GEMM tile. For tiles whose four 32-row subtiles are contiguous interior rows of one segment, the input rows plus a 2*dilation halo are staged once per channel slice into a double-buffered LDS region. All three taps then read from it at shifted offsets, instead of re-staging the A operand for every tap. This is meant to cut global-to-LDS traffic for the activation operand to roughly a third for dilations up to 32. It adds a per-block runtime eligibility check, a larger LDS footprint and new swizzled addressing, and is enabled by default with a toggle API.

```diff
diff --git a/include/radian_hip.h b/include/radian_hip.h
--- a/include/radian_hip.h
+++ b/include/radian_hip.h
@@ -53,6 +53,9 @@
 int rd_set_head_pack(rd_ctx* ctx, int on);
 int rd_head_pack_active(rd_ctx* ctx);
 int64_t rd_head_pack_tiles(rd_ctx* ctx);
+int rd_set_conv_slab(rd_ctx* ctx, int on);
+int rd_conv_slab_active(rd_ctx* ctx);
+int64_t rd_conv_slab_tiles(rd_ctx* ctx);
 
 int rd_forward(rd_ctx* ctx, const float* windows, int n_windows, int chunk_len, float* probs);
 
diff --git a/radian_amd/_lib.py b/radian_amd/_lib.py
--- a/radian_amd/_lib.py
+++ b/radian_amd/_lib.py
@@ -36,6 +36,9 @@
     "rd_set_head_pack": (c_i, [c_vp, c_i]),
     "rd_head_pack_active": (c_i, [c_vp]),
     "rd_head_pack_tiles": (c_i64, [c_vp]),
+    "rd_set_conv_slab": (c_i, [c_vp, c_i]),
+    "rd_conv_slab_active": (c_i, [c_vp]),
+    "rd_conv_slab_tiles": (c_i64, [c_vp]),
     "rd_set_decode_partition": (c_i, [c_vp, c_i]),
     "rd_forward": (c_i, [c_vp, c_vp, c_i, c_i, c_vp]),
     "rd_assemble": (c_i, [c_vp, c_vp, c_i, c_i, c_i, c_i, c_vp, c_i64, c_i64p, ctypes.POINTER(c_i)]),
diff --git a/radian_amd/backend.py b/radian_amd/backend.py
--- a/radian_amd/backend.py
+++ b/radian_amd/backend.py
@@ -868,6 +868,15 @@
 
     def head_pack_tiles(self):
         return int(self._L.rd_head_pack_tiles(self._h))
+
+    def set_conv_slab(self, on):
+        self._check(self._L.rd_set_conv_slab(self._h, 1 if on else 0))
+
+    def conv_slab_active(self):
+        return bool(self._L.rd_conv_slab_active(self._h))
+
+    def conv_slab_tiles(self):
+        return int(self._L.rd_conv_slab_tiles(self._h))
 
     def set_decode_form(self, form):
         self._check(self._L.rd_set_decode_form(self._h, {"auto": 0, "waves": 1, "lanes": 2, "two": 3, "one": 4, "queue": 5}[form] if isinstance(form, str) else int(form)))
diff --git a/radian_amd/csrc/common.h b/radian_amd/csrc/common.h
--- a/radian_amd/csrc/common.h
+++ b/radian_amd/csrc/common.h
@@ -101,6 +101,24 @@
     int32_t pad_;
 };
 
+constexpr int RD_SLAB_DMAX = 32;
+__host__ __device__ inline bool rd_slab_sub(const TileDesc& d0, const TileDesc& dj, int j)
+{
+    const int64_t end = (int64_t)d0.t0 + 128;
+    return (d0.t0 >= 0) & (end <= d0.seg_len) & (end <= d0.in_len) & (dj.seg_row == d0.seg_row) & (dj.t0 == d0.t0 + 32 * j) &
+           (dj.seg_len == d0.seg_len) & (dj.in_len == d0.in_len) & (dj.alt_in >= end) & (dj.alt_res >= end);
+}
+inline bool rd_slab_tile(const TileDesc* d)
+{
+    return rd_slab_sub(d[0], d[0], 0) && rd_slab_sub(d[0], d[1], 1) && rd_slab_sub(d[0], d[2], 2) && rd_slab_sub(d[0], d[3], 3);
+}
+inline int rd_count_slab_tiles(const TileDesc* list, size_t n_tiles)
+{
+    int n = 0;
+    for (size_t i = 0; i < n_tiles; i++) n += rd_slab_tile(list + 4 * i) ? 1 : 0;
+    return n;
+}
+
 constexpr int RD_MAX_LAYERS = 2 * 16 + 1;
 
 struct PackClass {
@@ -120,6 +138,8 @@
     int64_t rows[RD_MAX_LAYERS];
     const TileDesc* head_segs[RD_MAX_LAYERS];
     PackLayer pack[RD_MAX_LAYERS];
+    int slab[RD_MAX_LAYERS];
+    int slab_stream[RD_MAX_LAYERS];
 };
 
 struct KernelTimer {
@@ -148,6 +168,8 @@
     int conv_fuse = 1;
     int64_t packed_tiles = 0;
     int head_pack = 1;
+    int conv_slab = 1;
+    int64_t slab_tiles = 0;
     int conv_shape = 0;
     int logits_f16 = 0;
     hipStream_t stream = nullptr;
@@ -157,6 +179,7 @@
     LM lm;
     DevBuf ws_tiles, ws_raw;
     int tiles_nW = -1, tiles_T = -1;
+    int tiles_slab = 0;
     FwdLane lanes[2 * RD_MAX_LANES];
     int part_mode = -1;
     int part_cus = 0;
@@ -199,6 +222,7 @@
 void rd_lm_bind(LM& lm);
 int rd_lm_finish_device(rd_ctx* ctx, int table_order, int context_len, int hashed);
 bool rd_pack_heads(const rd_ctx* ctx);
+bool rd_conv_slab(const rd_ctx* ctx);
 int rd_forward_dev(rd_ctx* ctx, const float* d_windows, int nW, int T, float* d_probs, int lane = 0);
 int rd_forward_tiles_dev(rd_ctx* ctx, const float* d_signal, const TileLists& tiles, int64_t total_rows, void* d_probs, int lane = 0,
                          int probs_f16 = 0 );
diff --git a/radian_amd/csrc/context.hip b/radian_amd/csrc/context.hip
--- a/radian_amd/csrc/context.hip
+++ b/radian_amd/csrc/context.hip
@@ -259,6 +259,22 @@
 
 extern "C" int64_t rd_head_pack_tiles(rd_ctx* ctx) { return ctx ? ctx->packed_tiles : 0; }
 
+extern "C" int rd_set_conv_slab(rd_ctx* ctx, int on)
+{
+    RD_REQUIRE(ctx, "rd_set_conv_slab: null context");
+    RD_REQUIRE(on == 0 || on == 1, "rd_set_conv_slab: %d (1 = slab tiles stage their input rows once per channel slice, 0 = once per tap)", on);
+    ctx->conv_slab = on;
+    return RD_OK;
+}
+
+extern "C" int rd_conv_slab_active(rd_ctx* ctx)
+{
+    if (!ctx) return 0;
+    return rd_conv_slab(ctx) ? 1 : 0;
+}
+
+extern "C" int64_t rd_conv_slab_tiles(rd_ctx* ctx) { return ctx ? ctx->slab_tiles : 0; }
+
 extern "C" int rd_set_decode_partition(rd_ctx* ctx, int cus_per_xcd)
 {
     RD_REQUIRE(ctx, "rd_set_decode_partition: null context");
diff --git a/radian_amd/csrc/forward.hip b/radian_amd/csrc/forward.hip
--- a/radian_amd/csrc/forward.hip
+++ b/radian_amd/csrc/forward.hip
@@ -53,6 +53,7 @@
     PackClass cls[3];
     int n_heads;
     int n_stream;
+    int slab;
 };
 
 __device__ __forceinline__ float conv_in_value(float b, float w0, float w1, float w2, float x0, float x1, float x2)
@@ -172,22 +173,25 @@
     constexpr int FIN_FLOATS = FIN ? 2 * 4 * (32 + 2 * FIN_DMAX) * BK + 4 * RD_C : 0;
     return (EPI == EPI_HEAD && HEAD_FLOATS > 3 * STAGE_FLOATS) ? HEAD_FLOATS : 3 * STAGE_FLOATS + FIN_FLOATS;
 }
-template <int NT, int TAPS, int EPI, int WM, bool FIN, bool PACKED, int TAP_LO = 0>
+template <int NT, int TAPS, int EPI, int WM, bool FIN, bool PACKED, int TAP_LO = 0, bool SLAB = false>
 __device__ __forceinline__ void tcn_gemm_tile(const ConvArgs& a, float* const smem)
 {
+    static_assert(!SLAB || (NT == 4 && TAPS == 3 && (EPI == EPI_RELU || EPI == EPI_RES_IDENT) && WM == 2 && !FIN && !PACKED), "SLAB: the product shape's conv launches behind block 0");
     static_assert(!FIN || (EPI == EPI_RES_MATCH && WM == 2 && TAPS == 3 && NT == 4), "FIN: block 0's second conv, product shape");
     static_assert(!PACKED || (NT == 4 && TAPS == 3 && (EPI == EPI_RELU || EPI == EPI_RES_IDENT) && WM == 2 && !FIN), "PACKED: the product shape's conv launches behind block 0");
     constexpr int BM = 64 * WM;
     constexpr int NWAVE = 2 * WM;
     constexpr int BN = 2 * NT * 32;
     constexpr int NCHUNK = TAPS * (RD_C / BK);
-    constexpr int A_FLOATS = FIN ? 0 : BM * BK;
+    constexpr int A_FLOATS = (FIN || SLAB) ? 0 : BM * BK;
     constexpr int STAGE_FLOATS = A_FLOATS + BN * BK;
+    constexpr int SLAB_ROWS = BM + 2 * RD_SLAB_DMAX;
+    static_assert(!SLAB || 3 * STAGE_FLOATS + 2 * SLAB_ROWS * BK <= conv_smem_floats<NT, TAPS, EPI, WM, FIN>(), "SLAB: three weight stages and two regions fit the kernel's LDS block");
     constexpr int HEAD_FLOATS = BM * (RD_H + 1) + RD_H * 5 + 8 + BM * 5;
     constexpr int NSTAGE = 3;
     constexpr int MIDROWS = 4 * (32 + 2 * FIN_DMAX);
     constexpr int FIN_FLOATS = FIN ? 2 * MIDROWS * BK + 4 * RD_C : 0;
-    static_assert(conv_smem_floats<NT, TAPS, EPI, WM, FIN>() == ((EPI == EPI_HEAD && HEAD_FLOATS > NSTAGE * STAGE_FLOATS) ? HEAD_FLOATS : NSTAGE * STAGE_FLOATS + FIN_FLOATS),
+    static_assert(SLAB || conv_smem_floats<NT, TAPS, EPI, WM, FIN>() == ((EPI == EPI_HEAD && HEAD_FLOATS > NSTAGE * STAGE_FLOATS) ? HEAD_FLOATS : NSTAGE * STAGE_FLOATS + FIN_FLOATS),
                   "the kernel's LDS block");
 
     if constexpr (FIN) clear_zero_rows(a.zr);
@@ -208,8 +212,13 @@
         pk_p0 = (unsigned)((int)blockIdx.x - pkc.first_tile) * BM;
         pk_rows = (unsigned)a.n_heads * (unsigned)pkc.L;
     }
-    const bool mval[2] = {PACKED ? pk_p0 + wm * 64 < pk_rows : sdm[0].seg_len > sdm[0].t0,
-                          PACKED ? pk_p0 + wm * 64 + 32 < pk_rows : sdm[1].seg_len > sdm[1].t0};
+    const bool mval[2] = {SLAB || (PACKED ? pk_p0 + wm * 64 < pk_rows : sdm[0].seg_len > sdm[0].t0),
+                          SLAB || (PACKED ? pk_p0 + wm * 64 + 32 < pk_rows : sdm[1].seg_len > sdm[1].t0)};
+    int s_seg = 0, s_t0 = 0;
+    if constexpr (SLAB) {
+        s_seg = __builtin_amdgcn_readfirstlane((int)tds[0].seg_row);
+        s_t0 = __builtin_amdgcn_readfirstlane(tds[0].t0);
+    }
 
     const int dma_r = lane >> 2;
     const int dma_ps = lane & 3;
@@ -219,7 +228,16 @@
     const int d_len = sst.seg_len > sst.t0 ? sst.in_len : 0;
     const int lane_slot = (dma_ps ^ ((dma_r >> 2) & 3)) * 4;
     int arow[TAPS][2];
-    if constexpr (!PACKED) {
+    int srow[3] = {0, 0, 0};
+    const bool slab_p2 = SLAB && (8 + wave) * 16 < BM + 2 * a.dil;
+    if constexpr (SLAB) {
+#pragma unroll
+        for (int j = 0; j < 3; j++) {
+            const int r = (4 * j + wave) * 16 + dma_r;
+            const int t = s_t0 - 2 * a.dil + r;
+            srow[j] = (t >= 0 && r < BM + 2 * a.dil) ? s_seg + t : a.zero_row;
+        }
+    } else if constexpr (!PACKED) {
 #pragma unroll
         for (int tap = 0; tap < TAPS; tap++)
 #pragma unroll
@@ -249,7 +267,7 @@
     const unsigned lane_off = lane * 16;
 
     constexpr int PB = BN / (16 * NWAVE);
-    constexpr int NA = FIN ? 0 : 2;
+    constexpr int NA = (FIN || SLAB) ? 0 : 2;
     constexpr int NPIECE = NA + PB;
     auto stage_piece_at = [&](int chunk, int cc, int ar, float* st, int pc) {
         if (pc < NA) {
@@ -274,6 +292,11 @@
 #pragma unroll
         for (int pc = 0; pc < NPIECE; pc++) stage_piece_at(chunk, cc, arow[tap][pc & 1], st, pc);
     };
+    float* const slabb = smem + NSTAGE * STAGE_FLOATS;
+    auto slab_piece = [&](int cc, int reg, int j) {
+        const char* src = lanebase + (size_t)cc * (BK * 4) + (uint64_t)(unsigned)srow[j] * (RD_C * 4);
+        glds16_uncounted((const float*)src, slabb + reg * (SLAB_ROWS * BK) + (4 * j + wave) * 256);
+    };
 
     float* const midb = smem + NSTAGE * STAGE_FLOATS;
     float* const wins = midb + 2 * MIDROWS * BK;
@@ -337,7 +360,16 @@
     const int a_off = (wm * 64 + fr) * BK;
     const int b_off = A_FLOATS + (wn * NT * 32 + fr) * BK;
 
-    const bool work = mval[0] || mval[1];
+    const bool work = SLAB || mval[0] || mval[1];
+    int soff[3][BK / 8] = {{0, 0}, {0, 0}, {0, 0}};
+    if constexpr (SLAB) {
+#pragma unroll
+        for (int tap = 0; tap < 3; tap++) {
+            const int rr = wm * 64 + fr + tap * a.dil;
+#pragma unroll
+            for (int g = 0; g < BK / 8; g++) soff[tap][g] = rr * BK + (((2 * g + fh) ^ ((rr >> 2) & 3)) * 4);
+        }
+    }
     int frow[3][2] = {{0, 0}, {0, 0}, {0, 0}}, fswz[3][2] = {{0, 0}, {0, 0}, {0, 0}};
     if constexpr (FIN) {
 #pragma unroll
@@ -349,7 +381,8 @@
                 fswz[tap][m] = (rho >> 2) & 3;
             }
     }
-    auto chunk_step = [&](const float* st, int cur, int cur_tap, const bool st_ok, int next, int next_cc, int next_ar0, int next_ar1, float* nst) {
+    auto chunk_step = [&](const float* st, int cur, int cur_tap, const bool st_ok, int next, int next_cc, int next_ar0, int next_ar1, float* nst,
+                          const float* Rb = nullptr, const bool a_ok = false) {
         const float* Ab = st + a_off;
         const float* Bb = st + b_off;
         const float* Mb = midb + ((cur / TAPS) & 1) * (MIDROWS * BK);
@@ -359,6 +392,7 @@
 #pragma unroll
             for (int m = 0; m < 2; m++) {
                 if constexpr (FIN) af[g & 1][m] = *(const float4*)(Mb + frow[cur_tap][m] + (((2 * g + fh) ^ fswz[cur_tap][m]) * 4));
+                else if constexpr (SLAB) af[g & 1][m] = *(const float4*)(Rb + m * 32 * BK + soff[cur_tap][g]);
                 else af[g & 1][m] = *(const float4*)(Ab + m * 32 * BK + koff[g]);
             }
         };
@@ -387,7 +421,11 @@
                 __builtin_amdgcn_sched_group_barrier(0x008, 8, 0);
             }
             __builtin_amdgcn_sched_barrier(0);
-            if (st_ok && sidx < NPIECE) stage_piece_at(next, next_cc, sidx == 0 ? next_ar0 : next_ar1, nst, sidx);
+            if constexpr (SLAB) {
+                if (sidx == 0) {
+                    if (a_ok) slab_piece(next_cc, next_ar1, next_ar0);
+                } else if (st_ok && sidx <= NPIECE) stage_piece_at(next, 0, 0, nst, sidx - 1);
+            } else if (st_ok && sidx < NPIECE) stage_piece_at(next, next_cc, sidx == 0 ? next_ar0 : next_ar1, nst, sidx);
             if constexpr (FIN) {
                 if (sidx == NPIECE && cur / TAPS + 1 < RD_C / BK) fin_pass(cur / TAPS + 1, cur_tap);
             }
@@ -395,7 +433,7 @@
         }
     };
 
-    static_assert(NPIECE <= (BK / 8) * NT, "one DMA piece per MFMA step");
+    static_assert(NPIECE + (SLAB ? 1 : 0) <= (BK / 8) * NT, "one DMA piece per MFMA step");
     float* st0 = smem;
     float* st1 = smem + STAGE_FLOATS;
     float* st2 = smem + 2 * STAGE_FLOATS;
@@ -414,7 +452,31 @@
             if (chunk + 2 < NCHUNK) step(chunk + 2, T3 ? 2 : 0, st2, T3 ? 1 : 0, st1);
         }
     };
-    if constexpr (PACKED) {
+    if constexpr (SLAB) {
+        constexpr int NSL = RD_C / BK;
+        static_assert(NSL % 2 == 0, "the slab loop advances by the two regions");
+        slab_piece(0, 0, 0);
+        slab_piece(0, 0, 1);
+        if (slab_p2) slab_piece(0, 0, 2);
+#pragma unroll
+        for (int pc = 0; pc < NPIECE; pc++) stage_piece_at(0, 0, 0, st0, pc);
+#pragma unroll
+        for (int pc = 0; pc < NPIECE; pc++) stage_piece_at(1, 0, 0, st1, pc);
+        for (int s2 = 0; s2 < NSL; s2 += 2) {
+#pragma unroll
+            for (int h = 0; h < 2; h++) {
+                const int s = s2 + h;
+                const bool more = s + 1 < NSL;
+                const float* Rb = slabb + h * (SLAB_ROWS * BK);
+                wait_dma_and_barrier<NPIECE>();
+                chunk_step(st0, 0, 0, true, 3 * s + 2, s + 1, 0, 1 - h, st2, Rb, more);
+                if (more) wait_dma_and_barrier<NPIECE + 1>(); else wait_dma_and_barrier<NPIECE>();
+                chunk_step(st1, 0, 1, more, 3 * s + 3, s + 1, 1, 1 - h, st0, Rb, more);
+                if (more) wait_dma_and_barrier<NPIECE + 1>(); else wait_dma_and_barrier<0>();
+                chunk_step(st2, 0, 2, more, 3 * s + 4, s + 1, 2, 1 - h, st1, Rb, more && slab_p2);
+            }
+        }
+    } else if constexpr (PACKED) {
         constexpr int NTP = TAPS - TAP_LO, NCH = (RD_C / BK) * NTP, PERIOD = NTP == 2 ? 6 : 3;
         stage_piece_all(TAP_LO, 0, TAP_LO, st0);
         stage_piece_all((1 / NTP) * TAPS + TAP_LO + 1 % NTP, 1 / NTP, TAP_LO + 1 % NTP, st1);
@@ -505,17 +567,21 @@
 #pragma unroll
         for (int m = 0; m < 2; m++) {
             if (!mval[m]) continue;
-            const TileDesc sd = sdm[m];
+            TileDesc sd = sdm[m];
+            if constexpr (SLAB) {
+                sd.seg_row = s_seg;
+                sd.t0 = s_t0 + (wm * 2 + m) * 32;
+            }
             const int T = sd.seg_len;
             float* __restrict__ outw = a.out + (size_t)sd.seg_row * RD_C;
             const float* __restrict__ resw = a.resid + (size_t)sd.seg_row * RD_C;
             const float* __restrict__ resalt = a.resid + (size_t)sd.alt_row * RD_C;
-            const bool interior = sd.t0 + 32 <= T;
-            const bool res_one = EPI != EPI_RES_IDENT || sd.t0 + 32 <= sd.alt_res || sd.t0 >= sd.alt_res;
+            const bool interior = SLAB || sd.t0 + 32 <= T;
+            const bool res_one = SLAB || EPI != EPI_RES_IDENT || sd.t0 + 32 <= sd.alt_res || sd.t0 >= sd.alt_res;
             if (EPI != EPI_RES_MATCH && interior && res_one) {
                 const unsigned lbyte = (rrow * RD_C + c4) * 4;
                 float* __restrict__ ob = outw + (size_t)sd.t0 * RD_C + wn * (NT * 32);
-                const float* __restrict__ rb = (sd.t0 < sd.alt_res ? resw : resalt) + (size_t)sd.t0 * RD_C + wn * (NT * 32);
+                const float* __restrict__ rb = ((SLAB || sd.t0 < sd.alt_res) ? resw : resalt) + (size_t)sd.t0 * RD_C + wn * (NT * 32);
 #pragma unroll
                 for (int np = 0; np < NT / 2; np++) {
                     to_patch(m, np);
@@ -619,6 +685,14 @@
             else if (bx >= a.cls[1].first_tile) tcn_gemm_tile<NT, TAPS, EPI, WM, FIN, true, 1>(a, smem);
             else tcn_gemm_tile<NT, TAPS, EPI, WM, FIN, true, 0>(a, smem);
             return;
+        }
+        if (a.slab) {
+            const TileDesc* __restrict__ tds = (a.mixed && bx == a.n_stream - 1) ? a.mixed : a.tiles + (size_t)bx * 4;
+            const int j = (int)threadIdx.x & 3;
+            if (__all(rd_slab_sub(tds[0], tds[j], j))) {
+                tcn_gemm_tile<NT, TAPS, EPI, WM, FIN, false, 0, true>(a, smem);
+                return;
+            }
         }
     }
     tcn_gemm_tile<NT, TAPS, EPI, WM, FIN, false>(a, smem);
@@ -1356,7 +1430,7 @@
 
 int launch_layer(rd_ctx* ctx, hipStream_t st, int b, int kind , const TileDesc* tiles, int n,
                 double rows, int zero_row, const float* d_signal, float* Xin, float* Xout, float* MID, float* d_probs, int probs_f16,
-                const PackLayer* pk, const TileDesc* head_segs)
+                const PackLayer* pk, const TileDesc* head_segs, int slab_list, int slab_stream)
 {
     if (n <= 0) return RD_OK;
     Model& m = ctx->model;
@@ -1481,6 +1555,11 @@
         a.n_stream = pk->n_stream_tiles;
         n = pk->n_tiles;
         ctx->packed_tiles += pk->n_tiles - pk->n_stream_tiles;
+        slab_list = slab_stream;
+    }
+    if (b > 0 && a.dil <= RD_SLAB_DMAX && rd_conv_slab(ctx)) {
+        a.slab = 1;
+        ctx->slab_tiles += slab_list;
     }
     SplitArgs sa = {};
     sa.zero_row = zero_row;
@@ -1536,6 +1615,8 @@
 
 }
 
+bool rd_conv_slab(const rd_ctx* ctx) { return ctx->conv_slab && ctx->precision == 0 && ctx->conv_shape == 0; }
+
 bool rd_pack_heads(const rd_ctx* ctx)
 {
     return ctx->head_pack && ctx->precision == 0 && ctx->conv_shape == 0 && ctx->model.loaded && ctx->model.pack_ok;
@@ -1661,11 +1742,12 @@
     const int zero_row = (int)total_rows;
     const int nl = 2 * m.nblocks + 1;
     ctx->packed_tiles = 0;
+    ctx->slab_tiles = 0;
     for (int li = 0; li < nl; li++) {
         const int b = li == nl - 1 ? m.nblocks : li / 2;
         const int kind = li == nl - 1 ? 3 : (li == 0 ? 0 : (li & 1 ? 2 : 1));
         if ((rc = launch_layer(ctx, L->st, b, kind, tl.d[li], tl.n[li], (double)tl.rows[li], zero_row, d_signal, Xin, Xout, MID, (float*)d_probs, probs_f16,
-                               &tl.pack[li], tl.head_segs[li])))
+                               &tl.pack[li], tl.head_segs[li], tl.slab[li], tl.slab_stream[li])))
             return rc;
         if (kind == 2) {
             float* t = Xin;
@@ -1704,6 +1786,7 @@
         RD_HIP(hipMemcpy(ctx->ws_tiles.p, h.data(), h.size() * sizeof(TileDesc), hipMemcpyHostToDevice));
         ctx->tiles_nW = nW;
         ctx->tiles_T = T;
+        ctx->tiles_slab = rd_count_slab_tiles(h.data(), n);
     }
     const int nl = 2 * ctx->model.nblocks + 1;
     for (int li = 0; li < RD_MAX_LAYERS; li++) {
@@ -1712,6 +1795,8 @@
         out->rows[li] = li < nl ? (int64_t)nW * T : 0;
         out->head_segs[li] = nullptr;
         out->pack[li] = PackLayer();
+        out->slab[li] = li < nl ? ctx->tiles_slab : 0;
+        out->slab_stream[li] = 0;
     }
     return RD_OK;
 }
diff --git a/radian_amd/csrc/plan.hip b/radian_amd/csrc/plan.hip
--- a/radian_amd/csrc/plan.hip
+++ b/radian_amd/csrc/plan.hip
@@ -242,6 +242,7 @@
         lists.rows[li] = 0;
         lists.head_segs[li] = nullptr;
         lists.pack[li] = PackLayer();
+        lists.slab[li] = lists.slab_stream[li] = 0;
     }
     for (int li = 0; li < P.n_layers; li++) {
         if (P.per_layer || li == 0) {
@@ -250,11 +251,13 @@
             lists.d[li] = d_base + off;
             lists.n[li] = (int)(v.size() / 4);
             lists.rows[li] = P.rows[li];
+            lists.slab[li] = rd_count_slab_tiles(v.data(), v.size() / 4);
             off += v.size();
         } else {
             lists.d[li] = lists.d[0];
             lists.n[li] = lists.n[0];
             lists.rows[li] = lists.rows[0];
+            lists.slab[li] = lists.slab[0];
         }
     }
     return off;
@@ -274,10 +277,12 @@
         const std::vector<TileDesc>& v = P.head_segs[li];
         lists.head_segs[li] = nullptr;
         lists.pack[li] = PackLayer();
+        lists.slab_stream[li] = 0;
         if (v.empty() || P.pack[li].n_tiles == 0) continue;
         memcpy(h_dst + off, v.data(), v.size() * sizeof(TileDesc));
         lists.head_segs[li] = d_base + off;
         lists.pack[li] = P.pack[li];
+        lists.slab_stream[li] = rd_count_slab_tiles(P.tiles[li].data(), (size_t)(P.pack[li].n_stream_tiles - P.pack[li].mixed));
         off += v.size();
     }
     return off;
```

Result: faster. 27.95 million, median of 6 (+1.1%).
